# cgbur/llama2.zig

Measured on AMD Instinct MI355X. Metric: tokens/s (argmax, -t 0), higher is better.
Workload: dtype f32; 1 GPU; llama2-7b shape, fp32 llama2.c-v0 checkpoint (dim 4096, hidden 11008, L 32, H 32, kv 32, V 32000, S 2048), greedy from BOS, seeded synthetic weights; parallelism=1 GPU

## Files before the change

llama2.zig_amd/csrc/forward.cpp:

```cpp
#include <algorithm>
#include <cmath>
#include <cstdlib>
#include <cstring>
#include <mutex>

#include "batch_host.h"
#include "l2z_state.h"

namespace l2z {

struct Prof {
    std::vector<hipEvent_t> ev;
    std::vector<int> kind;
};

#define L2Z_LAUNCH(kind_id, expr)                                                         \
    do {                                                                                  \
        hipEvent_t _a = nullptr, _b = nullptr;                                            \
        if (prof) {                                                                       \
            L2Z_HIP(hipEventCreate(&_a));                                                 \
            L2Z_HIP(hipEventCreate(&_b));                                                 \
            L2Z_HIP(hipEventRecord(_a, st));                                              \
        }                                                                                 \
        L2Z_HIP(expr);                                                                    \
        if (prof) {                                                                       \
            L2Z_HIP(hipEventRecord(_b, st));                                              \
            prof->ev.push_back(_a);                                                       \
            prof->ev.push_back(_b);                                                       \
            prof->kind.push_back(kind_id);                                                \
        }                                                                                 \
    } while (0)

int check_pair(const l2z_config *config, const l2z_runstate *s, const l2z_weights *w, bool paged_ok)
{
    L2Z_CHECK(config && s && w, L2Z_ERR_INVALID, "null config / runstate / weights");
    L2Z_CHECK(paged_ok || s->pool == nullptr, L2Z_ERR_INVALID,
              "a paged runstate (l2z_runstate_init_paged) is taken by the wide family only: l2z_prefill_batch, "
              "l2z_transformer_wide, l2z_wide_run, l2z_verify_wide");
    L2Z_CHECK(memcmp(config, &s->cfg, sizeof *config) == 0 &&
                  memcmp(config, &w->cfg, sizeof *config) == 0,
              L2Z_ERR_INVALID, "config does not match the one RunState / Weights were built with");
    L2Z_CHECK(s->device == w->device && s->sh.rank == w->sh.rank && s->sh.world == w->sh.world,
              L2Z_ERR_INVALID, "RunState and Weights live on different devices / shards");
    L2Z_CHECK(s->sh.scheme_b == w->sh.scheme_b, L2Z_ERR_INVALID,
              "RunState and Weights were built under different sharding schemes (L2Z_SCHEME_B changed in between)");
    return L2Z_OK;
}

int enqueue_forward(l2z_runstate *s, const l2z_weights *w, StepKind step, Prof *prof,
                    int only_stage, int variant, int only_kind)
{
    const bool with_step = step != STEP_NONE;
    const bool split = variant == ATTN_SPLIT || variant == ATTN_SPLIT_S;
    const l2z_config &c = s->cfg;
    const Shard &sh = s->sh;
    hipStream_t st = s->stream;
    const l2z_comm *lc = s->comm;
    const size_t dim = c.dim, hid = c.hidden_dim;
    const int mb = s->max_blocks;
    int stage = 0;
    auto want = [&]() { return only_stage < 0 || only_stage == stage; };
    auto kind = [&](int k) { return only_kind < 0 || only_kind == k; };
    const bool p2p = s->d_push != nullptr && only_stage < 0 && sh.world > 1;
    const bool consume = p2p && s->ll_consume;
    const bool can_push = p2p && consume;
    const bool sb = sh.scheme_b;
    const bool xchg = step == STEP_GREEDY && p2p && s->xchg_steps;
    const int n_g = s->n_gathers;
    int gi = 0;
    bool pushed = false;
    const int *ctl = lc ? lc->d_ctl : nullptr;
    auto gather = [&](float *buf, size_t count_per_rank) -> int {
        stage++;
        gi++;
        if (only_stage >= 0 || only_kind >= 0) return L2Z_OK;
        const bool was_pushed = pushed;
        pushed = false;
        if (consume) {
            L2Z_CHECK(was_pushed, L2Z_ERR_STATE, "consumer-side gather %d: the producer did not push", gi);
            if (gi < n_g) return L2Z_OK;
        }
        hipEvent_t ea = nullptr, eb = nullptr;
        const bool timed = prof != nullptr && s->comm != nullptr && s->comm->world > 1;
        if (timed) {
            L2Z_HIP(hipEventCreate(&ea));
            L2Z_HIP(hipEventCreate(&eb));
            L2Z_HIP(hipEventRecord(ea, st));
        }
        L2Z_TRY(comm_allgather_inplace(s->comm, buf, count_per_rank, gi, n_g, was_pushed, st));
        if (timed) {
            L2Z_HIP(hipEventRecord(eb, st));
            prof->ev.push_back(ea);
            prof->ev.push_back(eb);
            prof->kind.push_back(KIND_GATHER);
        }
        return L2Z_OK;
    };
    auto reduce = [&]() -> int {
        stage++;
        gi++;
        if (only_stage >= 0 || only_kind >= 0) return L2Z_OK;
        const bool was_pushed = pushed;
        pushed = false;
        hipEvent_t ea = nullptr, eb = nullptr;
        if (prof != nullptr) {
            L2Z_HIP(hipEventCreate(&ea));
            L2Z_HIP(hipEventCreate(&eb));
            L2Z_HIP(hipEventRecord(ea, st));
        }
        L2Z_TRY(comm_allreduce(s->comm, s->part, s->x, dim, gi, was_pushed, st));
        if (prof != nullptr) {
            L2Z_HIP(hipEventRecord(eb, st));
            prof->ev.push_back(ea);
            prof->ev.push_back(eb);
            prof->kind.push_back(KIND_GATHER);
        }
        return L2Z_OK;
    };
    auto x_in = [&](MatvecArgs &a, const float *plain, int g, size_t count_per_rank) {
        a.x = plain;
        if (consume && g >= 1) a.xin = comm_ll_in(s->comm, g, count_per_rank);
    };
    auto push_to = [&](MatvecArgs &a, int which) {
        if (!can_push) return;
        a.push = s->d_push + which;
        a.push_ctl = ctl;
        a.push_gi = comm_gi(lc, gi + 1);
    };
    auto col_shard = [&](MatvecArgs &a, const float *wcols, const float *x_loc, int n_pad, int *epi) {
        a.w0 = wcols;
        a.x = x_loc;
        a.n = n_pad;
        a.rows0 = c.dim;
        a.out0 = s->part;
        a.resid = sh.rank == 0 ? s->x : nullptr;
        *epi = sh.rank == 0 ? EPI_RESID : EPI_STORE;
        push_to(a, 1);
    };
    const bool pk = s->packed_w && w->pk_blob != nullptr && !sb && sh.world == 1 && !consume;
    for (int l = 0; l < c.n_layers; l++) {
        float *kc = s->key_cache + (size_t)l * c.seq_len * sh.kvd_loc;
        float *vc = s->value_cache + (size_t)l * c.seq_len * sh.kvd_loc;
        const size_t kvh_stride = (size_t)c.seq_len * sh.hs;
        const bool fused = s->fused_qkv_attn && !split && only_stage < 0;
        if (fused && kind(KIND_QKV)) {
            FusedQkvAttnArgs a = {};
            a.wq = w->wq + (size_t)l * dim * dim;
            a.wk = w->wk + (size_t)l * dim * dim;
            a.wv = w->wv + (size_t)l * dim * dim;
            a.rms_w = w->rms_att + (size_t)l * dim; a.x = s->x; a.q_out = s->q;
            a.kcache = kc; a.vcache = vc; a.xb = s->xb; a.pos_ptr = s->d_pos; a.rope = s->rope;
            a.n = c.dim; a.head_size = sh.hs; a.seq_len = c.seq_len; a.kv_dim = sh.kvd_loc;
            a.kv_row = sh.hs; a.kv_head = kvh_stride;
            L2Z_LAUNCH(KIND_QKV, launch_fused_qkv_attn(a, c.n_heads, st));
        }
        if (!fused && want() && kind(KIND_QKV)) {
            MatvecArgs a = {};
            a.w0 = w->wq + (size_t)l * sh.dim_loc * dim;
            a.w1 = w->wk + (size_t)l * sh.kvd_loc * dim;
            a.w2 = w->wv + (size_t)l * sh.kvd_loc * dim;
            a.out0 = s->q; a.out1 = kc; a.out2 = vc;
            a.rows0 = sh.dim_loc; a.rows1 = sh.kvd_loc; a.rows2 = sh.kvd_loc;
            a.pos_stride1 = sh.hs; a.pos_stride2 = sh.hs; a.kv_head_stride = kvh_stride;
            a.n = c.dim; a.rms_w = w->rms_att + (size_t)l * dim;
            x_in(a, s->x, gi, sh.dim_loc);
            a.pos_ptr = s->d_pos; a.rope = s->rope; a.head_size = sh.hs; a.rope_segs = 2;
            L2Z_LAUNCH(KIND_QKV, launch_matvec(a, PRO_RMS, EPI_ROPE, mb, g_cus, st));
        }
        if (!fused && want() && kind(KIND_ATTN)) {
            AttnArgs a = {};
            a.q = s->q; a.kcache = kc; a.vcache = vc; a.xb = s->xb + sh.dim0;
            a.pos_ptr = s->d_pos; a.head_size = sh.hs; a.kv_row = sh.hs; a.kv_head = kvh_stride;
            a.kv_mul = c.n_heads / c.n_kv_heads; a.seq_len = c.seq_len;
            a.tl_seq = s->tl_attn_seq++;
            if (!sb && can_push && attention_push_supported(a)) {
                a.push = s->d_push + 0;
                a.push_ctl = ctl;
                a.push_gi = comm_gi(lc, gi + 1);
                pushed = true;
            }
            if (split && s->attn_nch > 1 && attention_split_supported(a))
                L2Z_LAUNCH(KIND_ATTN, launch_attention_split(a, sh.heads_loc, s->attn_nch,
                                                             s->d_attn_part, s->d_attn_cnt, st, variant == ATTN_SPLIT_S));
            else
                L2Z_LAUNCH(KIND_ATTN, launch_attention(a, sh.heads_loc, st, variant == ATTN_SHORT ? 1 : 0));
        }
        if (!sb) L2Z_TRY(gather(s->xb, sh.dim_loc));
        if (want() && kind(KIND_WO)) {
            MatvecArgs a = {};
            int epi = EPI_RESID;
            if (sb) {
                col_shard(a, w->wo + (size_t)l * dim * sh.dimc_pad, s->xb + sh.dim0, sh.dimc_pad, &epi);
            } else {
                a.w0 = w->wo + (size_t)l * sh.dim_loc * dim;
                a.out0 = s->x + sh.dim0; a.resid = s->x + sh.dim0;
                a.rows0 = sh.dim_loc; a.n = c.dim;
                x_in(a, s->xb, gi, sh.dim_loc);
                push_to(a, 1);
            }
            L2Z_LAUNCH(KIND_WO, launch_matvec(a, PRO_NONE, epi, mb, g_cus, st, nullptr, &pushed));
        }
        if (sb) L2Z_TRY(reduce());
        else L2Z_TRY(gather(s->x, sh.dim_loc));
        if (want() && kind(KIND_FFN13)) {
            MatvecArgs a = {};
            a.w0 = w->w1 + (size_t)l * sh.hid_loc * 2 * dim;
            a.w1 = w->w3 + (size_t)l * sh.hid_loc * 2 * dim;
            a.out0 = sb ? s->hb : s->hb + sh.hid0;
            a.rows0 = sh.hid_loc; a.rows1 = sh.hid_loc; a.n = c.dim;
            a.rms_w = w->rms_ffn + (size_t)l * dim;
            x_in(a, s->x, gi, sh.dim_loc);
            if (!sb) push_to(a, 2);
            if (pk && w->pk[l].p != nullptr) { a.pk = w->pk[l].p; a.pk_e = w->pk[l].e; }
            L2Z_LAUNCH(KIND_FFN13, launch_matvec(a, PRO_RMS, EPI_SWIGLU, mb, g_cus, st, nullptr, &pushed));
        }
        if (!sb) L2Z_TRY(gather(s->hb, sh.hid_loc));
        if (want() && kind(KIND_FFN2)) {
            MatvecArgs a = {};
            int epi = EPI_RESID;
            if (sb) {
                col_shard(a, w->w2 + (size_t)l * dim * sh.hidc_pad, s->hb, sh.hidc_pad, &epi);
            } else {
                a.w0 = w->w2 + (size_t)l * sh.dim_loc * hid;
                a.out0 = s->x + sh.dim0; a.resid = s->x + sh.dim0;
                a.rows0 = sh.dim_loc; a.n = c.hidden_dim;
                x_in(a, s->hb, gi, sh.hid_loc);
                push_to(a, 1);
            }
            L2Z_LAUNCH(KIND_FFN2, launch_matvec(a, PRO_NONE, epi, mb, g_cus, st, nullptr, &pushed));
        }
        if (sb) L2Z_TRY(reduce());
        else L2Z_TRY(gather(s->x, sh.dim_loc));
    }
    if (want() && kind(KIND_CLS)) {
        MatvecArgs a = {};
        a.w0 = w->wcls; a.out0 = s->logits + sh.v0;
        a.rows0 = sh.v_loc; a.n = c.dim; a.rms_w = w->rms_final;
        x_in(a, s->x, gi, sh.dim_loc);
        a.part_val = s->d_part_val; a.part_idx = s->d_part_idx; a.row_offset = sh.v0;
        const bool fuse = (sh.world == 1 || xchg || (only_kind >= 0 && with_step && s->comm && !s->comm->nccl && !s->comm->p2p)) &&
                          matvec_vector_width(c.dim);
        int grid = 0;
        if (!xchg) push_to(a, 3);
        L2Z_LAUNCH(KIND_CLS, launch_matvec(a, PRO_RMS, fuse ? EPI_ARGMAX : EPI_STORE, mb, g_cus, st,
                                           &grid, &pushed));
        s->n_part = fuse ? grid : 0;
        if (only_stage < 0 && only_kind < 0) (with_step ? s->n_part_step : s->n_part_fwd) = s->n_part;
    }
    if (xchg) {
        stage++;
        gi++;
        pushed = false;
        if (only_kind < 0) s->logits_partial = true;
    } else {
        L2Z_TRY(gather(s->logits, sh.v_loc));
    }
    if (step == STEP_GREEDY && want() && kind(KIND_ARGMAX)) {
        ArgmaxArgs a = {};
        a.logits = s->logits; a.vocab = c.vocab_size; a.token_ptr = s->d_token;
        if (s->n_part > 0) { a.part_val = s->d_part_val; a.part_idx = s->d_part_idx; a.n_part = s->n_part; }
        a.pos_ptr = s->d_pos; a.prompt = s->d_prompt; a.n_prompt_ptr = s->d_n_prompt;
        a.out_tokens = s->d_out_tokens; a.argmax_out = s->d_argmax; a.tok_emb = w->tok_emb;
        a.x = s->x; a.dim = c.dim; a.advance = 1;
        if (xchg && only_kind < 0) {
            a.xchg = s->d_push + 3;
            a.xchg_gi = comm_gi(lc, n_g);
            a.epoch_ctl = lc->d_ctl;
            a.epoch_add = lc->solo ? 0 : n_g;
        }
        L2Z_LAUNCH(KIND_ARGMAX, launch_argmax(a, st));
    }
    if (step == STEP_SAMPLE && want() && kind(KIND_ARGMAX)) {
        L2Z_CHECK(sh.world == 1 && s->d_smp_ctl != nullptr && s->d_smp_scratch != nullptr, L2Z_ERR_STATE,
                  "sampled step on a runstate l2z_sample_run has not prepared");
        SampleStepArgs a = {};
        a.logits = s->logits; a.vocab = c.vocab_size; a.seq_len = c.seq_len;
        a.params = (const SampleStepParams *)s->d_smp_ctl; a.coins = s->d_smp_ctl + 2; a.scratch = s->d_smp_scratch;
        a.token_ptr = s->d_token; a.pos_ptr = s->d_pos; a.prompt = s->d_prompt; a.n_prompt_ptr = s->d_n_prompt;
        a.out_tokens = s->d_out_tokens; a.tok_emb = w->tok_emb; a.x = s->x; a.dim = c.dim;
        L2Z_LAUNCH(KIND_ARGMAX, launch_sample_step(a, st));
    }
    return L2Z_OK;
}

int attn_variant(const l2z_runstate *s, int pos)
{
    if (s->attn_nch > 1 && pos >= s->attn_split_pos) return pos < s->attn_split_wide_pos ? ATTN_SPLIT_S : ATTN_SPLIT;
    return pos < s->attn_short_pos ? ATTN_SHORT : ATTN_HEAD;
}

int build_graph(l2z_runstate *s, const l2z_weights *w, StepKind step, int variant,
                hipGraphExec_t *out)
{
    hipGraph_t graph = nullptr;
    L2Z_HIP(hipStreamBeginCapture(s->stream, hipStreamCaptureModeThreadLocal));
    int rc = enqueue_forward(s, w, step, nullptr, -1, variant);
    hipError_t e = hipStreamEndCapture(s->stream, &graph);
    if (rc != L2Z_OK) {
        if (graph) (void)hipGraphDestroy(graph);
        return rc;
    }
    L2Z_HIP(e);
    e = hipGraphInstantiate(out, graph, nullptr, nullptr, 0);
    (void)hipGraphDestroy(graph);
    L2Z_HIP(e);
    return L2Z_OK;
}

void drop_graphs(l2z_runstate *s)
{
    for (int v = 0; v < ATTN_VARIANTS; v++) {
        if (s->g_forward[v]) { (void)hipGraphExecDestroy(s->g_forward[v]); s->g_forward[v] = nullptr; }
        if (s->g_step[v]) { (void)hipGraphExecDestroy(s->g_step[v]); s->g_step[v] = nullptr; }
        if (s->g_sample[v]) { (void)hipGraphExecDestroy(s->g_sample[v]); s->g_sample[v] = nullptr; }
    }
    s->graph_w_uid = 0;
}

hipGraphExec_t *graph_slot(l2z_runstate *s, StepKind step, int variant)
{
    return step == STEP_SAMPLE ? &s->g_sample[variant] : step == STEP_GREEDY ? &s->g_step[variant] : &s->g_forward[variant];
}

int ensure_graph(l2z_runstate *s, const l2z_weights *w, int variant, StepKind step)
{
    if (!s->use_graphs) return L2Z_OK;
    int rc = L2Z_OK;
    if (s->graph_w_uid != w->uid) {
        drop_graphs(s);
        s->graph_w_uid = w->uid;
        const int edges[] = {0, s->attn_short_pos, s->attn_split_pos, s->attn_split_wide_pos, s->cfg.seq_len};
        bool reach[ATTN_VARIANTS] = {};
        for (int e : edges)
            for (int p = e - 1; p <= e; p++)
                if (p >= 0 && p < s->cfg.seq_len) reach[attn_variant(s, p)] = true;
        for (int v = 0; v < ATTN_VARIANTS && rc == L2Z_OK; v++) {
            if (!reach[v]) continue;
            rc = build_graph(s, w, STEP_NONE, v, &s->g_forward[v]);
            if (rc == L2Z_OK) rc = build_graph(s, w, STEP_GREEDY, v, &s->g_step[v]);
        }
    }
    hipGraphExec_t *slot = graph_slot(s, step, variant);
    if (rc == L2Z_OK && *slot) return L2Z_OK;
    if (rc != L2Z_OK || build_graph(s, w, step, variant, slot) != L2Z_OK) {
        fprintf(stderr, "llama2_hip: hipGraph capture failed (%s); launching eagerly\n", l2z_last_error());
        drop_graphs(s);
        s->use_graphs = false;
        (void)hipGetLastError();
    }
    return L2Z_OK;
}

int run_forward(l2z_runstate *s, const l2z_weights *w, StepKind step, int pos)
{
    const bool with_step = step != STEP_NONE;
    const int variant = attn_variant(s, pos);
    L2Z_CHECK(s->sh.world == 1 || (s->comm && (s->comm->nccl || s->comm->p2p)), L2Z_ERR_STATE,
              "sharded runstate without a transport: connect the group (RCCL id or "
              "l2z_comm_p2p_export/_connect), or drive emulated ranks with l2z_emu_transformer");
    L2Z_TRY(comm_check(s->comm));
    L2Z_TRY(ensure_graph(s, w, variant, step));
    s->logits_partial = step == STEP_GREEDY && s->xchg_steps && s->d_push != nullptr && s->sh.world > 1;
    if (s->use_graphs) {
        s->n_part = with_step ? s->n_part_step : s->n_part_fwd;
        L2Z_HIP(hipGraphLaunch(*graph_slot(s, step, variant), s->stream));
        return L2Z_OK;
    }
    return enqueue_forward(s, w, step, nullptr, -1, variant);
}

int ensure_logits(l2z_runstate *s)
{
    if (!s->logits_partial) return L2Z_OK;
    L2Z_TRY(comm_allgather_inplace(s->comm, s->logits, (size_t)s->sh.v_loc, 1, 1, false, s->stream));
    s->logits_partial = false;
    s->n_part = 0;
    return L2Z_OK;
}


}

using namespace l2z;

extern "C" int l2z_transformer(int token, int pos, const l2z_config *config, l2z_runstate *s,
                               const l2z_weights *w)
{
    L2Z_TRY(check_pair(config, s, w));
    L2Z_CHECK(token >= 0 && token < config->vocab_size, L2Z_ERR_STATE, "token %d out of range", token);
    L2Z_CHECK(pos >= 0 && pos < config->seq_len, L2Z_ERR_STATE, "pos %d out of range [0,%d)", pos,
              config->seq_len);
    L2Z_HIP(hipSetDevice(s->device));
    L2Z_HIP(launch_set_state(token, pos, s->d_token, s->d_pos, w->tok_emb, s->x, config->dim,
                             s->stream));
    L2Z_TRY(run_forward(s, w, STEP_NONE, pos));
    s->host_pos = pos + 1;
    return L2Z_OK;
}

extern "C" int l2z_argmax(l2z_runstate *s, int *out_token)
{
    L2Z_CHECK(s && out_token, L2Z_ERR_INVALID, "l2z_argmax: null argument");
    L2Z_HIP(hipSetDevice(s->device));
    L2Z_TRY(ensure_logits(s));
    ArgmaxArgs a = {};
    a.logits = s->logits; a.vocab = s->cfg.vocab_size; a.argmax_out = s->d_argmax; a.advance = 0;
    if (s->n_part > 0) { a.part_val = s->d_part_val; a.part_idx = s->d_part_idx; a.n_part = s->n_part; }
    L2Z_HIP(launch_argmax(a, s->stream));
    L2Z_HIP(hipMemcpyAsync(out_token, s->d_argmax, sizeof(int), hipMemcpyDeviceToHost, s->stream));
    L2Z_HIP(hipStreamSynchronize(s->stream));
    return L2Z_OK;
}

extern "C" int l2z_logits_read(l2z_runstate *s, float *out_logits)
{
    L2Z_CHECK(s && out_logits, L2Z_ERR_INVALID, "l2z_logits_read: null argument");
    L2Z_HIP(hipSetDevice(s->device));
    L2Z_TRY(ensure_logits(s));
    L2Z_HIP(hipMemcpyAsync(out_logits, s->logits, (size_t)s->cfg.vocab_size * sizeof(float),
                           hipMemcpyDeviceToHost, s->stream));
    L2Z_HIP(hipStreamSynchronize(s->stream));
    L2Z_TRY(comm_check(s->comm));
    return L2Z_OK;
}

extern "C" int l2z_probs_read(l2z_runstate *s, float temperature, float *out_probs)
{
    L2Z_CHECK(s && out_probs, L2Z_ERR_INVALID, "l2z_probs_read: null argument");
    L2Z_CHECK(temperature > 0.0f, L2Z_ERR_INVALID, "l2z_probs_read: temperature %g (0 is the argmax path)", (double)temperature);
    L2Z_HIP(hipSetDevice(s->device));
    L2Z_TRY(ensure_logits(s));
    if (s->d_probs == nullptr) L2Z_HIP(hipMalloc(&s->d_probs, (size_t)s->cfg.vocab_size * sizeof(float)));
    L2Z_HIP(launch_probs(s->d_probs, s->logits, s->cfg.vocab_size, temperature, s->stream));
    const size_t bytes = (size_t)s->cfg.vocab_size * sizeof(float);
    if (s->h_stage == nullptr) L2Z_HIP(hipHostMalloc((void **)&s->h_stage, bytes, hipHostMallocDefault));
    L2Z_HIP(hipMemcpyAsync(s->h_stage, s->d_probs, bytes, hipMemcpyDeviceToHost, s->stream));
    L2Z_HIP(hipStreamSynchronize(s->stream));
    L2Z_TRY(comm_check(s->comm));
    memcpy(out_probs, s->h_stage, bytes);
    return L2Z_OK;
}

extern "C" int l2z_greedy_begin(l2z_runstate *s, const int32_t *prompt, int n_prompt)
{
    L2Z_CHECK(s != nullptr && n_prompt >= 0 && (n_prompt == 0 || prompt != nullptr),
              L2Z_ERR_INVALID, "l2z_greedy_begin: bad arguments");
    L2Z_CHECK(n_prompt <= s->cfg.seq_len, L2Z_ERR_INVALID, "prompt longer than seq_len");
    L2Z_CHECK(s->pool == nullptr, L2Z_ERR_INVALID, "l2z_greedy_begin: a paged runstate is taken by the wide family only");
    for (int i = 0; i < n_prompt; i++)
        L2Z_CHECK(prompt[i] >= 0 && prompt[i] < s->cfg.vocab_size, L2Z_ERR_INVALID,
                  "prompt[%d] = %d out of vocabulary", i, prompt[i]);
    L2Z_HIP(hipSetDevice(s->device));
    L2Z_HIP(hipStreamSynchronize(s->stream));
    if (n_prompt)
        L2Z_HIP(hipMemcpy(s->d_prompt, prompt, (size_t)n_prompt * sizeof(int), hipMemcpyHostToDevice));
    L2Z_HIP(hipMemcpy(s->d_n_prompt, &n_prompt, sizeof(int), hipMemcpyHostToDevice));
    s->h_prompt.assign(prompt, prompt + n_prompt);
    s->host_pos = 0;
    s->done = false;
    return L2Z_OK;
}

namespace l2z {
namespace {

int step_loop(const l2z_config *config, l2z_runstate *s, const l2z_weights *w, int n_steps, StepKind step,
              int32_t *out_tokens, int *out_n)
{
    *out_n = 0;
    L2Z_HIP(hipSetDevice(s->device));
    if (s->done) return L2Z_OK;
    int remaining = n_steps;
    if (remaining > config->seq_len - s->host_pos) remaining = config->seq_len - s->host_pos;
    if (remaining <= 0) return L2Z_OK;
    if (s->host_pos == 0) {
        L2Z_HIP(launch_set_state(1, 0, s->d_token, s->d_pos, w->tok_emb, s->x, config->dim,
                                 s->stream));
    }
    const int kChunk = 64;
    int produced = 0;
    const int np = (int)s->h_prompt.size();
    if (s->host_pos == 0 && np >= kPrefillMinPrompt && remaining >= np && prefill_enabled() &&
        prefill_usable(s) &&
        std::find(s->h_prompt.begin(), s->h_prompt.end(), 1) == s->h_prompt.end()) {
        std::vector<int32_t> in((size_t)np);
        in[0] = 1;
        for (int i = 1; i < np; i++) in[(size_t)i] = s->h_prompt[(size_t)i - 1];
        L2Z_TRY(prefill_tokens(s, w, in.data(), np, 0));
        L2Z_HIP(hipMemcpyAsync(s->d_out_tokens, s->d_prompt, (size_t)np * sizeof(int),
                               hipMemcpyDeviceToDevice, s->stream));
        L2Z_HIP(launch_set_state(s->h_prompt[(size_t)np - 1], np, s->d_token, s->d_pos, w->tok_emb,
                                 s->x, config->dim, s->stream));
        for (int i = 0; i < np; i++) out_tokens[i] = s->h_prompt[(size_t)i];
        produced = np;
        s->host_pos = np;
        remaining -= np;
    }
    while (remaining > 0 && !s->done) {
        const int n = remaining < kChunk ? remaining : kChunk;
        for (int i = 0; i < n; i++) L2Z_TRY(run_forward(s, w, step, s->host_pos + i));
        L2Z_HIP(hipMemcpyAsync(out_tokens + produced, s->d_out_tokens + s->host_pos,
                               (size_t)n * sizeof(int), hipMemcpyDeviceToHost, s->stream));
        L2Z_HIP(hipStreamSynchronize(s->stream));
        L2Z_TRY(comm_check(s->comm));
        int got = n;
        for (int i = 0; i < n; i++) {
            if (out_tokens[produced + i] == 1) {
                got = i + 1;
                s->done = true;
                break;
            }
        }
        produced += got;
        s->host_pos += got;
        remaining -= n;
    }
    *out_n = produced;
    return L2Z_OK;
}

}
}

extern "C" int l2z_greedy_run(const l2z_config *config, l2z_runstate *s, const l2z_weights *w,
                              int n_steps, int32_t *out_tokens, int *out_n)
{
    L2Z_TRY(check_pair(config, s, w));
    L2Z_CHECK(out_tokens && out_n && n_steps >= 0, L2Z_ERR_INVALID, "l2z_greedy_run: bad arguments");
    return step_loop(config, s, w, n_steps, STEP_GREEDY, out_tokens, out_n);
}

extern "C" int l2z_sample_run(const l2z_config *config, l2z_runstate *s, const l2z_weights *w, int n_steps,
                              float temperature, float top_p, const float *coins, int32_t *out_tokens, int *out_n)
{
    L2Z_TRY(no_device_check());
    L2Z_CHECK(out_tokens && out_n && n_steps >= 0, L2Z_ERR_INVALID, "l2z_sample_run: bad arguments");
    L2Z_TRY(check_pair(config, s, w));
    L2Z_CHECK(s->comm == nullptr && s->sh.world == 1, L2Z_ERR_INVALID,
              "l2z_sample_run: the runstate is a shard (a shard holds its own rows of the logits only)");
    L2Z_TRY(check_draw("l2z_sample_run", -1, temperature, top_p, coins));
    if (temperature > 0.0f) L2Z_TRY(check_coins("l2z_sample_run", coins, 0, n_steps));
    *out_n = 0;
    const int left = config->seq_len - s->host_pos;
    const int n = n_steps < left ? n_steps : left;
    if (s->done || n <= 0) return L2Z_OK;
    L2Z_HIP(hipSetDevice(s->device));
    const size_t ctl_bytes = (2 + (size_t)config->seq_len) * sizeof(float);
    if (s->d_smp_ctl == nullptr) {
        L2Z_HIP(hipMalloc((void **)&s->d_smp_ctl, ctl_bytes));
        L2Z_HIP(hipMemset(s->d_smp_ctl, 0, ctl_bytes));
    }
    if (s->h_smp_ctl == nullptr) L2Z_HIP(hipHostMalloc((void **)&s->h_smp_ctl, ctl_bytes, hipHostMallocDefault));
    if (s->d_smp_scratch == nullptr)
        L2Z_HIP(hipMalloc((void **)&s->d_smp_scratch, sample_scratch_floats(config->vocab_size) * sizeof(float)));
    s->h_smp_ctl[0] = temperature;
    s->h_smp_ctl[1] = top_p;
    L2Z_HIP(hipMemcpyAsync(s->d_smp_ctl, s->h_smp_ctl, 2 * sizeof(float), hipMemcpyHostToDevice, s->stream));
    if (temperature > 0.0f) {
        float *h = s->h_smp_ctl + 2 + s->host_pos;
        memcpy(h, coins, (size_t)n * sizeof(float));
        L2Z_HIP(hipMemcpyAsync(s->d_smp_ctl + 2 + s->host_pos, h, (size_t)n * sizeof(float), hipMemcpyHostToDevice, s->stream));
    }
    return step_loop(config, s, w, n_steps, STEP_SAMPLE, out_tokens, out_n);
}

extern "C" int l2z_profile_forward(int token, int pos, const l2z_config *config, l2z_runstate *s,
                                   const l2z_weights *w, double *ms_by_kind, int *launches_by_kind,
                                   int n_kinds)
{
    L2Z_TRY(check_pair(config, s, w));
    L2Z_CHECK(ms_by_kind && launches_by_kind && n_kinds >= KIND_COUNT, L2Z_ERR_INVALID,
              "l2z_profile_forward: need %d kind slots", (int)KIND_COUNT);
    L2Z_CHECK(token >= 0 && token < config->vocab_size && pos >= 0 && pos < config->seq_len,
              L2Z_ERR_STATE, "token/pos out of range");
    L2Z_HIP(hipSetDevice(s->device));
    L2Z_HIP(launch_set_state(token, pos, s->d_token, s->d_pos, w->tok_emb, s->x, config->dim,
                             s->stream));
    Prof prof;
    int rc = enqueue_forward(s, w, STEP_GREEDY, &prof, -1, attn_variant(s, pos));
    hipError_t e = hipStreamSynchronize(s->stream);
    for (int k = 0; k < n_kinds; k++) { ms_by_kind[k] = 0.0; launches_by_kind[k] = 0; }
    if (rc == L2Z_OK && e == hipSuccess) {
        for (size_t i = 0; i < prof.kind.size(); i++) {
            float ms = 0.0f;
            if (hipEventElapsedTime(&ms, prof.ev[2 * i], prof.ev[2 * i + 1]) == hipSuccess) {
                ms_by_kind[prof.kind[i]] += ms;
                launches_by_kind[prof.kind[i]] += 1;
            }
        }
    }
    for (hipEvent_t ev : prof.ev) (void)hipEventDestroy(ev);
    s->host_pos = pos + 1;
    if (rc != L2Z_OK) return rc;
    L2Z_HIP(e);
    return L2Z_OK;
}

extern "C" int l2z_time_kind(int kind, int pos, const l2z_config *config, l2z_runstate *s,
                             const l2z_weights *w, int reps, double *avg_ms_per_launch, int *launches)
{
    L2Z_TRY(check_pair(config, s, w));
    L2Z_CHECK(kind >= 0 && kind < KIND_GATHER && avg_ms_per_launch && reps >= 1, L2Z_ERR_INVALID,
              "l2z_time_kind: bad arguments");
    L2Z_CHECK(s->sh.world == 1 || (s->comm && ((!s->comm->nccl && !s->comm->p2p) || s->comm->solo)), L2Z_ERR_INVALID,
              "l2z_time_kind: unsharded runstates, emulated or solo ranks only (a connected shard would wait for its peers)");
    L2Z_CHECK(pos >= 0 && pos < config->seq_len, L2Z_ERR_STATE, "pos out of range");
    L2Z_HIP(hipSetDevice(s->device));
    L2Z_HIP(launch_set_state(1, pos, s->d_token, s->d_pos, w->tok_emb, s->x, config->dim, s->stream));
    hipEvent_t e0, e1;
    L2Z_HIP(hipEventCreate(&e0));
    L2Z_HIP(hipEventCreate(&e1));
    const int per_pass = kind == KIND_CLS || kind == KIND_ARGMAX ? 1 : config->n_layers;
    int rc = enqueue_forward(s, w, STEP_GREEDY, nullptr, -1, attn_variant(s, pos), kind);
    hipError_t e = hipEventRecord(e0, s->stream);
    for (int r = 0; r < reps && rc == L2Z_OK; r++) rc = enqueue_forward(s, w, STEP_GREEDY, nullptr, -1, attn_variant(s, pos), kind);
    if (e == hipSuccess) e = hipEventRecord(e1, s->stream);
    if (e == hipSuccess) e = hipEventSynchronize(e1);
    float ms = 0.0f;
    if (e == hipSuccess) e = hipEventElapsedTime(&ms, e0, e1);
    (void)hipEventDestroy(e0);
    (void)hipEventDestroy(e1);
    hipError_t e2 = launch_set_state(1, pos, s->d_token, s->d_pos, w->tok_emb, s->x, config->dim, s->stream);
    if (e2 == hipSuccess) e2 = hipStreamSynchronize(s->stream);
    if (rc != L2Z_OK) return rc;
    L2Z_HIP(e);
    L2Z_HIP(e2);
    *avg_ms_per_launch = (double)ms / (double)(reps * per_pass);
    if (launches) *launches = reps * per_pass;
    return L2Z_OK;
}

extern "C" int l2z_emu_transformer(int n_ranks, l2z_runstate *const *ss,
                                   const l2z_weights *const *ws, int token, int pos)
{
    L2Z_CHECK(n_ranks >= 1 && ss && ws, L2Z_ERR_INVALID, "l2z_emu_transformer: bad arguments");
    const l2z_config &c = ss[0]->cfg;
    for (int r = 0; r < n_ranks; r++) {
        L2Z_TRY(check_pair(&c, ss[r], ws[r]));
        L2Z_CHECK(ss[r]->sh.world == n_ranks && ss[r]->sh.rank == r, L2Z_ERR_INVALID,
                  "l2z_emu_transformer: runstate %d is not rank %d of %d", r, r, n_ranks);
        L2Z_HIP(launch_set_state(token, pos, ss[r]->d_token, ss[r]->d_pos, ws[r]->tok_emb, ss[r]->x,
                                 c.dim, ss[r]->stream));
    }
    const bool sb = ss[0]->sh.scheme_b;
    const int n_stages = (sb ? 2 : 4) * c.n_layers + 1;
    for (int stage = 0; stage < n_stages; stage++) {
        for (int r = 0; r < n_ranks; r++)
            L2Z_TRY(enqueue_forward(ss[r], ws[r], STEP_NONE, nullptr, stage, attn_variant(ss[r], pos)));
        for (int r = 0; r < n_ranks; r++) L2Z_HIP(hipStreamSynchronize(ss[r]->stream));
        if (sb && stage < n_stages - 1) {
            const float *parts[kMaxWorld];
            L2Z_CHECK(n_ranks <= kMaxWorld, L2Z_ERR_INVALID, "l2z_emu_transformer: more than %d ranks", kMaxWorld);
            for (int r = 0; r < n_ranks; r++) parts[r] = ss[r]->part;
            for (int r = 0; r < n_ranks; r++) L2Z_HIP(launch_sum_parts(ss[r]->x, parts, n_ranks, c.dim, nullptr));
            L2Z_HIP(hipDeviceSynchronize());
            continue;
        }
        const Shard &sh0 = ss[0]->sh;
        size_t count;
        int which;
        if (stage == n_stages - 1) { which = 3; count = sh0.v_loc; }
        else if (stage % 4 == 0) { which = 0; count = sh0.dim_loc; }
        else if (stage % 4 == 2) { which = 2; count = sh0.hid_loc; }
        else { which = 1; count = sh0.dim_loc; }
        auto buf = [&](l2z_runstate *s) {
            return which == 0 ? s->xb : which == 1 ? s->x : which == 2 ? s->hb : s->logits;
        };
        for (int src = 0; src < n_ranks; src++)
            for (int dst = 0; dst < n_ranks; dst++)
                if (dst != src)
                    L2Z_HIP(hipMemcpy(buf(ss[dst]) + (size_t)src * count,
                                      buf(ss[src]) + (size_t)src * count, count * sizeof(float),
                                      hipMemcpyDeviceToDevice));
        L2Z_HIP(hipDeviceSynchronize());
    }
    for (int r = 0; r < n_ranks; r++) ss[r]->host_pos = pos + 1;
    return L2Z_OK;
}

extern "C" int l2z_kind_name(int kind, char *out, size_t cap)
{
    L2Z_CHECK(kind >= 0 && kind < KIND_COUNT && out && cap, L2Z_ERR_INVALID, "l2z_kind_name: bad kind");
    snprintf(out, cap, "%s", kKindNames[kind]);
    return L2Z_OK;
}
```

llama2.zig_amd/csrc/l2z_internal.h:

```cpp
#pragma once

#include <hip/hip_runtime.h>

#include <cstdarg>
#include <cstdint>
#include <cstdio>
#include <string>
#include <vector>

#include "../../include/llama2_hip.h"
#include "../../include/llama2_hip_test.h"

namespace l2z {

struct P2pArgs;

struct LLIn {
    const unsigned long long *slots;
    unsigned slot_floats;
    unsigned count;
    int gi;
    int *ctl;
    int *h_err;
    long long timeout_ticks;
};

void set_error(const char *fmt, ...);

#define L2Z_HIP(expr)                                                                    \
    do {                                                                                 \
        hipError_t _e = (expr);                                                          \
        if (_e != hipSuccess) {                                                          \
            ::l2z::set_error("%s failed: %s (%s:%d)", #expr, hipGetErrorString(_e),      \
                             __FILE__, __LINE__);                                        \
            return _e == hipErrorOutOfMemory ? L2Z_ERR_OOM                               \
                   : (_e == hipErrorNoDevice || _e == hipErrorInvalidDevice)             \
                       ? L2Z_ERR_NO_DEVICE                                               \
                       : L2Z_ERR_HIP;                                                    \
        }                                                                                \
    } while (0)

#define L2Z_CHECK(cond, code, ...)          \
    do {                                    \
        if (!(cond)) {                      \
            ::l2z::set_error(__VA_ARGS__);  \
            return (code);                  \
        }                                   \
    } while (0)

#define L2Z_TRY(expr)              \
    do {                           \
        int _s = (expr);           \
        if (_s != L2Z_OK) return _s; \
    } while (0)

template <class Sig> class FnRef;
template <class R, class... Args> class FnRef<R(Args...)> {
  public:
    template <class F>
    FnRef(const F &f) : f_(&f), call_([](const void *p, Args... args) -> R { return (*(const F *)p)(args...); }) {}
    R operator()(Args... args) const { return call_(f_, args...); }

  private:
    const void *f_;
    R (*call_)(const void *, Args...);
};


enum Prologue { PRO_NONE = 0, PRO_RMS = 1 };
enum Epilogue { EPI_STORE = 0, EPI_ROPE = 1, EPI_RESID = 2, EPI_SWIGLU = 3, EPI_ARGMAX = 4 };

constexpr int kMaxSeg = 3;

struct ArgmaxArgs {
    const float *logits;
    int vocab;
    const float *part_val;
    const int *part_idx;
    int n_part;
    int *token_ptr;
    int *pos_ptr;
    const int *prompt;
    const int *n_prompt_ptr;
    int *out_tokens;
    int *argmax_out;
    const float *tok_emb;
    float *x;
    int dim;
    int advance;
    int *epoch_ctl;
    int epoch_add;
    const P2pArgs *xchg;
    int xchg_gi;
};

struct MatvecArgs {
    const float *w0, *w1, *w2;
    float *out0, *out1, *out2;
    int rows0, rows1, rows2;
    int pos_stride1, pos_stride2;
    size_t kv_head_stride;
    int n;
    const float *x;
    const float *rms_w;
    const float *resid;
    const int *pos_ptr;
    const float2 *rope;
    int head_size;
    int rope_segs;
    float *part_val;
    int *part_idx;
    int row_offset;
    const P2pArgs *push;
    const int *push_ctl;
    int push_gi;
    LLIn xin;
    const uint32_t *pk;
    int pk_e;
};

struct AttnArgs {
    const float *q;
    const float *kcache;
    const float *vcache;
    float *xb;
    const int *pos_ptr;
    int head_size;
    int kv_row;
    size_t kv_head;
    int kv_mul;
    int seq_len;
    const P2pArgs *push;
    const int *push_ctl;
    int push_gi;
    int tl_seq;
};


struct FusedQkvAttnArgs {
    const float *wq, *wk, *wv;
    const float *rms_w, *x;
    float *q_out;
    float *kcache, *vcache;
    float *xb;
    const int *pos_ptr;
    const float2 *rope;
    int n;
    int head_size, seq_len, kv_dim;
    int kv_row;
    size_t kv_head;
};
bool fused_qkv_attn_supported(int dim, int n_heads, int n_kv_heads, int seq_len, int n_cus);
hipError_t launch_fused_qkv_attn(const FusedQkvAttnArgs &a, int n_heads, hipStream_t st);

hipError_t launch_pk_stats(const float *m, size_t count, uint32_t *stats, hipStream_t st);
hipError_t launch_pk_pack(const float *m, int rows, int n, int e_base, uint32_t *pk, hipStream_t st);
hipError_t launch_pk_unpack(const uint32_t *pk, int rows, int n, int e_base, float *out, hipStream_t st);
hipError_t launch_matvec(const MatvecArgs &a, int pro, int epi, int max_blocks_per_cu, int n_cus,
                         hipStream_t st, int *out_grid = nullptr, bool *pushed = nullptr);
bool attention_push_supported(const AttnArgs &a);
int matvec_max_grid(int n_cus);
bool matvec_vector_width(int n);
hipError_t launch_stream_read(const float *p, size_t n_floats, float *out, int n_cus, hipStream_t st);
hipError_t launch_attention(const AttnArgs &a, int n_heads_local, hipStream_t st, int form = 0);
int attention_short_pos(int head_size, int seq_len);
int attention_split_chunks(int n_heads_local, int n_cus);
size_t attention_split_part_floats(int n_heads_local, int head_size, int nch);
bool attention_split_supported(const AttnArgs &a);
hipError_t launch_attention_split(const AttnArgs &a, int n_heads_local, int nch, float *part,
                                  int *arrivals, hipStream_t st, bool small = false);
int attention_split_wide_pos(int seq_len);
hipError_t launch_argmax(const ArgmaxArgs &a, hipStream_t st);
hipError_t launch_set_state(int token, int pos, int *token_ptr, int *pos_ptr, const float *tok_emb,
                            float *x, int dim, hipStream_t st);
hipError_t launch_rmsnorm(float *o, const float *x, const float *w, int n, hipStream_t st);
hipError_t launch_softmax(float *x, int n, hipStream_t st);
hipError_t launch_probs(float *probs, const float *logits, int n, float temperature, hipStream_t st);
hipError_t launch_dot(float *out, const float *x, const float *y, int n, hipStream_t st);
hipError_t launch_weighted_sum_rows(float *xout, int xout_len, const float *rows, int row_stride,
                                    const float *weights, int n_weights, hipStream_t st);
hipError_t launch_synth_fill(float *dst, uint64_t base_idx, uint64_t count, uint64_t seed,
                             float scale, float bias, hipStream_t st, uint64_t row_len = 0, uint64_t row_pitch = 0,
                             uint64_t idx_pitch = 0);
hipError_t launch_sum_parts(float *out, const float *const *parts, int n_parts, int n, hipStream_t st);
hipError_t launch_copy_rows(float *dst, size_t dpitch, const float *src, size_t rows, size_t cols, hipStream_t st);
size_t attention_lds_bytes(int head_size, int seq_len, bool vec);

struct SplitKWs {
    float *part;
    int *cnt;
    size_t part_floats;
    int cnt_ints;
    void *x3;
    size_t x3_bytes;
    void *x3b;
    size_t x3b_bytes;
};
struct DeferredSum {
    const float *part;
    int sk, feat, tm;
    bool valid;
};
enum PlanesReady { PLANES_SPLIT = 0, PLANES_READY = 1, PLANES_READY_B = 2 };
constexpr int kSplitKMaxTokens = 256;
constexpr int kPanelWsRows = 6 * kSplitKMaxTokens;
int prefill_split_k(long long n_whole, int P, int K, bool pair);
enum PrefillGemmEpi { PG_STORE = 0, PG_RESID = 1, PG_ROPE = 2, PG_ROPE_CACHE = 3, PG_CACHE = 4,
                      PG_SWIGLU = 5 };
bool x3_applies(long long n_whole, int K);
bool x3_stream_shape(long long n_whole, int P, int K);
int x3_stream_sk(long long n_whole, int P, int K);
enum GemmKind { GEMM_SINGLE = 0,
                GEMM_QKV,
                GEMM_W13,
                GEMM_KV };
struct GemmShape {
    int kind, epi;
    int P, N, K, ldx;
    int n_scale;
    long long n_launch_whole;
    int sk;
    int nq, nkv;
    int w13_one_matrix;
    size_t part_floats;
    int cnt_ints;
};
enum GemmFamily { GF_INVALID = -1, GF_NOT_SUPPORTED = -2, GF_NO_WORKSPACE = -3,
                  GF_STREAM = 1,
                  GF_SHORT,
                  GF_SPLIT_K,
                  GF_TWO_BLOCK,
                  GF_TILE };
enum TileForm { TILE_128x64 = 0, TILE_64x64, TILE_32x64, TILE_32x32, TILE_128x128 };
struct GemmPlan {
    int family;
    int epi;
    int K;
    int x3;
    int sk;
    int tile;
    int feat, tm, nbuf, one_round;
    int tms, paired;
};
GemmPlan prefill_gemm_plan(const GemmShape &s);
hipError_t launch_prefill_rmsnorm(float *o, int ldo, const float *x, const float *w, int n, int P,
                                  hipStream_t st,
                                  void *x3 = nullptr, int kp = 0,
                                  const DeferredSum *pending = nullptr,
                                  const int *rows = nullptr);
hipError_t launch_prefill_embed(float *x, const float *tok_emb, const int *tokens, int dim, int P,
                                hipStream_t st);
hipError_t launch_prefill_attention(const float *q, int ldq, const float *kcache, const float *vcache,
                                    float *out, int ldo, int pos0, int P, int n_heads, int head_size,
                                    int kv_row, size_t kv_head, int kv_mul, int seq_len, hipStream_t st,
                                    int n_heads_model = 0,
                                    int form = 0,
                                    void *x3 = nullptr, int kp = 0,
                                    bool *planes_written = nullptr);
constexpr int kRaggedMaxSeq = 16;
struct RaggedSeq {
    float *kc, *vc;
    int row0, rows;
    int pos0;
    int pad;
    const int32_t *pages;
};
__device__ __forceinline__ int kv_page_id(const int32_t *pages, int i)
{
    return ((const __attribute__((address_space(4))) int32_t *)pages)[i];
}
struct RaggedLayer {
    const float *q;
    int ldq;
    float *out;
    int ldo;
    int P, n_heads, head_size, kv_mul, seq_len;
    size_t layer_off, kv_head_stride;
    hipStream_t st;
    void *x3;
    int kp;
};
using RaggedAttention = FnRef<hipError_t(const RaggedLayer &, bool *planes_written)>;
struct RaggedChunk {
    const RaggedSeq *seq;
    const int *row_seq;
    const int *row_pos;
    const int2 *tiles;
    int n_seq, n_tiles;
    int seq_max;
    float *k, *v;
    size_t page_floats;
    const RaggedAttention *attention;
    const int *att_rows;
    int n_att_rows;
};
hipError_t launch_ragged_rope_scatter(float *q, int ldq, const RaggedChunk &rg, int P, int dim, int kv_dim, int head_size,
                                      const float2 *rope, size_t layer_off, size_t kv_head_stride, hipStream_t st);
hipError_t launch_ragged_attention(const RaggedLayer &L, const RaggedChunk &rg, bool *planes_written = nullptr);
enum PanelEpi { PANEL_STORE = 0, PANEL_RESID = 1, PANEL_SWIGLU = 2, PANEL_QKV = 3 };
struct PanelProduct {
    const float *x;
    int ldx;
    const float *w0, *w1, *w2;
    int rows0, rows1, rows2;
    int P, K;
    int mode;
    float *out;
    int ldo;
    const float *res;
    int ldres;
    float *outk, *outv;
    int ldkv, head_size, pos0;
    size_t kv_head_stride;
    const float2 *rope;
};
bool prefill_panel_shape(long long n_whole, int P, int K, long long widest_whole);
int prefill_panel_max_tokens();
int prefill_next_chunk_of(const l2z_config &c, int remaining);
hipError_t launch_prefill_panel(const PanelProduct &p, int n_cus, const SplitKWs *ws, hipStream_t st);
int prefill_tile_form(int N, int P, int pair);
constexpr int kScoreSeg = 4096;
struct ScoreArgs {
    const float *slab;
    int ld, n, col0, P;
    const int *targets;
    float *part_m, *part_s;
    int *part_i;
    float *tgt;
    int seg0, nseg;
    float *out_logprob;
    int *out_top1;
};
hipError_t launch_score_reduce(const ScoreArgs &a, hipStream_t st);
hipError_t launch_score_finish(const ScoreArgs &a, hipStream_t st);
size_t matvec_lds_bytes(int n);

}
```

llama2.zig_amd/csrc/l2z_state.h:

```cpp
#pragma once
#include <cstdint>
#include <vector>

#include "kv_pages.h"
#include "l2z_comm.h"
#include "l2z_internal.h"
#include "tunables.h"

namespace l2z {

struct BatchScratch;
struct WideScratch;

struct Shard {
    int rank = 0, world = 1;
    int hs = 0;
    int dim0 = 0, dim_loc = 0;
    int kvd_loc = 0;
    int heads_loc = 0;
    int hid0 = 0, hid_loc = 0;
    int v0 = 0, v_loc = 0;
    bool scheme_b = false;
    int dimc_pad = 0, hidc_pad = 0;
};
int pad_cols(int n);
int make_shard(const l2z_config &c, const l2z_comm *comm, Shard *out);

enum ShardKind { REPL, BY_Q_HEADS, BY_KV_HEADS, BY_HIDDEN, BY_DIM_ROWS, BY_VOCAB, SKIP };

struct TensorDesc {
    const char *name;
    size_t offset;
    size_t layers, rows, cols;
    ShardKind kind;
    float scale, bias;
    size_t count() const { return layers * rows * cols; }
};
std::vector<TensorDesc> tensor_table(const l2z_config &c, bool shared);
void shard_rows(const TensorDesc &d, const Shard &s, size_t *r0, size_t *r1);

extern int g_cus;
int ensure_device(int device);
int current_device_for(const l2z_comm *comm);

}

struct l2z_weights {
    uint64_t uid = 0;
    l2z_config cfg;
    int shared;
    int device;
    l2z::Shard sh;
    float *blob = nullptr;
    size_t blob_floats = 0;
    bool file_layout = false;
    std::vector<size_t> dev_off;
    const float *tok_emb = nullptr, *rms_att = nullptr, *rms_ffn = nullptr, *rms_final = nullptr;
    const float *wq = nullptr, *wk = nullptr, *wv = nullptr, *wo = nullptr;
    const float *w1 = nullptr, *w2 = nullptr, *w3 = nullptr, *wcls = nullptr;
    struct PkMat {
        const uint32_t *p = nullptr;
        int e = 0;
    };
    uint32_t *pk_blob = nullptr;
    std::vector<PkMat> pk;
    int pk_packed = 0, pk_candidates = 0;
};

struct l2z_kvpool {
    l2z_config cfg;
    int device = 0;
    l2z::KvPages alloc;
    float *k = nullptr, *v = nullptr;
    size_t page_floats = 0;
    int live = 0;
};

enum { KIND_QKV = 0, KIND_ATTN, KIND_WO, KIND_FFN13, KIND_FFN2, KIND_CLS, KIND_ARGMAX, KIND_GATHER, KIND_COUNT };
static const char *const kKindNames[KIND_COUNT] = {"qkv", "attn", "wo", "ffn13", "ffn2", "cls", "argmax", "gather"};
static_assert(KIND_COUNT == L2Z_N_KINDS, "include/llama2_hip_test.h L2Z_N_KINDS");

struct l2z_runstate {
    l2z_config cfg;
    int device;
    l2z::Shard sh;
    const l2z_comm *comm = nullptr;
    hipStream_t stream = nullptr;
    float *x = nullptr, *xb = nullptr, *hb = nullptr, *q = nullptr, *logits = nullptr;
    float *part = nullptr;
    float *key_cache = nullptr, *value_cache = nullptr;
    l2z_kvpool *pool = nullptr;
    l2z::KvSeq pg;
    int32_t *d_pages = nullptr, *h_pages = nullptr;
    bool pages_dirty = false;
    float2 *rope = nullptr;
    int *d_token = nullptr, *d_pos = nullptr, *d_prompt = nullptr, *d_n_prompt = nullptr;
    int *d_out_tokens = nullptr, *d_argmax = nullptr;
    float *pf_x = nullptr, *pf_xn = nullptr, *pf_q = nullptr, *pf_att = nullptr;
    float *pf_h1 = nullptr;
    int pf_ld_xn = 0, pf_ld_att = 0, pf_ld_h1 = 0;
    float *pf_stage = nullptr;
    float *pf_part = nullptr;
    int *pf_tokens = nullptr;
    l2z::DeferredSum pf_pending = {nullptr, 1, 128, 1, false};
    l2z::PlanesReady pf_planes_att = l2z::PLANES_SPLIT, pf_planes_h1 = l2z::PLANES_SPLIT;
    l2z::SplitKWs pf_sk = {nullptr, nullptr, 0, 0, nullptr, 0, nullptr, 0};
    int pf_cap = 0;
    void *sc_ws = nullptr, *sc_seq = nullptr;
    size_t sc_ws_bytes = 0;
    int sc_cap = 0, sc_slab_n = 0;
    int sc_slab_force = 0;
    float *d_probs = nullptr;
    float *h_stage = nullptr;
    float *d_smp_ctl = nullptr, *h_smp_ctl = nullptr, *d_smp_scratch = nullptr;
    float *d_part_val = nullptr;
    int *d_part_idx = nullptr;
    int n_part = 0;
    int n_part_step = 0, n_part_fwd = 0;
    float *d_attn_part = nullptr;
    int *d_attn_cnt = nullptr;
    int attn_nch = 0;
    int attn_split_pos = 0;
    int attn_short_pos = 0;
    int attn_split_wide_pos = 0;
    uint64_t graph_w_uid = 0;
    hipGraphExec_t g_forward[4] = {nullptr, nullptr, nullptr, nullptr}, g_step[4] = {nullptr, nullptr, nullptr, nullptr};
    hipGraphExec_t g_sample[4] = {nullptr, nullptr, nullptr, nullptr};
    bool use_graphs = true;
    int host_pos = 0;
    bool done = false;
    std::vector<int32_t> h_prompt;
    l2z::P2pArgs *d_push = nullptr;
    int n_gathers = 0;
    bool ll_consume = false;
    bool xchg_steps = false;
    bool logits_partial = false;
    bool fused_qkv_attn = false;
    int max_blocks = 0;
    bool packed_w = true;
    int tl_attn_seq = 0;
    l2z::BatchScratch *bt = nullptr;
    float *rg_k = nullptr, *rg_v = nullptr;
    void *rg_tab = nullptr;
    int rg_cap = 0;
    l2z::WideScratch *wd = nullptr;
};

namespace l2z {

struct Prof;
int check_pair(const l2z_config *config, const l2z_runstate *s, const l2z_weights *w, bool paged_ok = false);
enum { ATTN_SHORT = 0, ATTN_HEAD = 1, ATTN_SPLIT_S = 2, ATTN_SPLIT = 3, ATTN_VARIANTS = 4 };
enum StepKind { STEP_NONE = 0, STEP_GREEDY = 1, STEP_SAMPLE = 2 };
int enqueue_forward(l2z_runstate *s, const l2z_weights *w, StepKind step, Prof *prof, int only_stage,
                    int variant, int only_kind = -1);
int attn_variant(const l2z_runstate *s, int pos);
int run_forward(l2z_runstate *s, const l2z_weights *w, StepKind step, int pos);
int ensure_logits(l2z_runstate *s);
void drop_graphs(l2z_runstate *s);

constexpr int kPrefillMinPrompt = L2Z_PREFILL_MIN_PROMPT;
bool prefill_enabled();
bool prefill_usable(const l2z_runstate *s);
bool prefill_shard_takes_the_unsharded_kernels(const l2z_config &c, const Shard &sh);
int prefill_check(const l2z_config *config, const l2z_runstate *s);
struct ScoreCall;
int prefill_tokens(l2z_runstate *s, const l2z_weights *w, const int32_t *tokens, int n_tokens, int pos0,
                   const ScoreCall *score = nullptr);

int prefill_scratch(l2z_runstate *s, int need);
int prefill_ragged_chunk(l2z_runstate *s, const l2z_weights *w, const int32_t *tokens, int P, const RaggedChunk &rg);
int prefill_last_logits(l2z_runstate *s, const l2z_weights *w);
int prefill_rows_logits(l2z_runstate *s, const l2z_weights *w, int P, float *out, int ldo, const int *rows = nullptr);
int ragged_alloc(l2z_runstate *s, int need);

int kv_check_kind(const char *fn, int n, l2z_runstate *const *states);
int kv_attach(const char *fn, int n, l2z_runstate *const *states, const int32_t *pos0, const int32_t *counts, int count);
int kv_upload(int n, l2z_runstate *const *states, hipStream_t st);
void kv_seq_base(const l2z_runstate *s, RaggedSeq *q);
inline size_t kv_page_floats(const l2z_runstate *s) { return s->pool != nullptr ? s->pool->page_floats : 0; }
int kv_release(l2z_runstate *s, int n_pos);
int kv_copy_rows(l2z_runstate *dst, const l2z_runstate *src, int r0, int n_pos);
void kv_runstate_free(l2z_runstate *s);

void batch_free(l2z_runstate *s);
void wide_free(l2z_runstate *s);
const float *wide_verify_row(const l2z_runstate *s, int row);
void wide_verify_forget(l2z_runstate *s);

}
```

llama2.zig_amd/csrc/matvec.hip:

```cpp
#include <type_traits>

#include "argmax_rule.h"
#include "matvec_device.h"
#include "packed_w.h"

namespace l2z {
namespace {

__device__ __forceinline__ void dot2_scalar(const float *__restrict__ pa,
                                            const float *__restrict__ pb, const float *xs, int n,
                                            float &ra, float &rb)
{
    const int lane = threadIdx.x & 63;
    float sa = 0.0f, sb = 0.0f;
    for (int j = lane; j < n; j += kWave) {
        const float xv = xs[j];
        sa = fmaf(pa[j], xv, sa);
        sb = fmaf(pb[j], xv, sb);
    }
    ra = wave_sum(sa);
    rb = wave_sum(sb);
}

template <int LPR>
struct MvGeom {
    static constexpr int RW = kWave / LPR;
    static constexpr int U = (LPR == 64) ? 4 : 6;
};

template <int LPR>
__device__ __forceinline__ void mv_load(const float *pa, const float *pb, int c0, int n4,
                                        v4f (&wa)[MvGeom<LPR>::U], v4f (&wb)[MvGeom<LPR>::U])
{
    constexpr int U = MvGeom<LPR>::U;
    const v4f *a4 = (const v4f *)pa, *b4 = (const v4f *)pb;
#pragma unroll
    for (int k = 0; k < U; k++) {
        int c = c0 + LPR * k;
        c = c < n4 ? c : n4 - 1;
        wa[k] = ldg_nt(a4 + c);
        wb[k] = ldg_nt(b4 + c);
    }
}

template <int LPR>
__device__ __forceinline__ void mv_consume(const v4f *xs4, int c0, const v4f (&wa)[MvGeom<LPR>::U],
                                           const v4f (&wb)[MvGeom<LPR>::U], v4f &acc_a, v4f &acc_b)
{
    constexpr int U = MvGeom<LPR>::U;
#pragma unroll
    for (int k = 0; k < U; k++) {
        const v4f xv = xs4[c0 + LPR * k];
        acc_a = fma4(wa[k], xv, acc_a);
        acc_b = fma4(wb[k], xv, acc_b);
    }
}

struct MvStep {
    bool unit_done, more;
    int u_next, b_next;
};

__device__ __forceinline__ MvStep mv_step(int u, int b, int n_batches, int ustride, int n_units)
{
    MvStep s;
    s.unit_done = (b + 1 == n_batches);
    s.u_next = s.unit_done ? u + ustride : u;
    s.b_next = s.unit_done ? 0 : b + 1;
    s.more = s.u_next < n_units;
    return s;
}

template <int PRO, int EPI, int LPR, int XC, bool LL>
__global__ __launch_bounds__(kBlock) void matvec_kernel(const MatvecArgs a)
{
    using G = MvGeom<LPR>;
    constexpr int U = G::U, RW = G::RW;
    extern __shared__ __attribute__((aligned(16))) float lds[];
    const MvLocals m = mv_locals<EPI>(a);
    const int n4 = m.n >> 2;
    const int n_batches = (n4 + LPR * U - 1) / (LPR * U);
    const int n4_pad = n_batches * (LPR * U);
    float *xs = lds;
    float *scratch = lds + 4 * n4_pad;
    const v4f *xs4 = (const v4f *)xs;

    const int lane = threadIdx.x & 63, wave = threadIdx.x >> 6;
    const int grp = lane / LPR, cl = lane % LPR;
    const int n_units = (m.n_pairs + RW - 1) / RW;
    const int ustride = gridDim.x * kWaves;

    XStage<PRO, XC, LL> xst;
    xst.issue(a.x, a.xin, a.rms_w, n4);
    int u = blockIdx.x * kWaves + wave;
    const bool has_unit = u < n_units;
    const float *pa, *pb;
    pair_rows<EPI>(m, (has_unit ? u : 0) * RW + grp, pa, pb);
    v4f wa[U], wb[U];
    EpiIn ein = epi_prefetch<EPI>(m, (has_unit ? u : 0) * RW + grp, cl == 0 && has_unit);
    EpiIn ein_next = ein;
    mv_load<LPR>(pa, pb, cl, n4, wa, wb);
    xst.finish(a.x, a.rms_w, m.n, n4_pad, xs, scratch);
    if (EPI != EPI_ARGMAX && !has_unit) return;

    v4f acc_a = {0.f, 0.f, 0.f, 0.f}, acc_b = {0.f, 0.f, 0.f, 0.f};
    ArgmaxCand best;
    int b = 0;
    while (has_unit) {
        mv_consume<LPR>(xs4, cl + b * (LPR * U), wa, wb, acc_a, acc_b);
        const MvStep s = mv_step(u, b, n_batches, ustride, n_units);
        if (s.more) {
            if (s.unit_done) {
                pair_rows<EPI>(m, s.u_next * RW + grp, pa, pb);
                ein_next = epi_prefetch<EPI>(m, s.u_next * RW + grp, cl == 0);
            }
            mv_load<LPR>(pa, pb, cl + s.b_next * (LPR * U), n4, wa, wb);
        }
        if (s.unit_done) {
            const float sa = lanes_sum(hsum4(acc_a), LPR);
            const float sb = lanes_sum(hsum4(acc_b), LPR);
            pair_epilogue<EPI>(m, u * RW + grp, sa, sb, cl == 0, ein);
            ein = ein_next;
            if (EPI == EPI_ARGMAX) {
                const int ra_ = 2 * (u * RW + grp), rb_ = ra_ + 1;
                if (ra_ < m.total_rows) argmax_take(best, sa, ra_ + a.row_offset);
                if (rb_ < m.total_rows) argmax_take(best, sb, rb_ + a.row_offset);
            }
            acc_a = v4f{0.f, 0.f, 0.f, 0.f};
            acc_b = v4f{0.f, 0.f, 0.f, 0.f};
        }
        if (!s.more) break;
        u = s.u_next;
        b = s.b_next;
    }
    if (EPI == EPI_ARGMAX) {
        argmax_wave_fold(best);
        __syncthreads();
        if (lane == 0) {
            scratch[wave] = best.v;
            scratch[kWaves + wave] = __int_as_float(best.i);
        }
        __syncthreads();
        if (threadIdx.x == 0) {
            ArgmaxCand c = {scratch[0], __float_as_int(scratch[kWaves])};
            for (int w = 1; w < kWaves; w++) argmax_merge(c, scratch[w], __float_as_int(scratch[kWaves + w]));
            a.part_val[blockIdx.x] = c.v;
            a.part_idx[blockIdx.x] = c.i;
        }
    }
}

struct PkRaw {
    v4u q4[7];
    uint32_t q1[3];
};

__device__ __forceinline__ void pk_load_raw(const uint32_t *src, int lane, int s, PkRaw &r)
{
    const int q = pk::lane_dw(s) / 4, rem = pk::lane_dw(s) % 4;
#pragma unroll
    for (int i = 0; i < 7; i++)
        if (i < q) r.q4[i] = __builtin_nontemporal_load((const v4u *)(src + i * 256 + lane * 4));
#pragma unroll
    for (int i = 0; i < 3; i++)
        if (i < rem) r.q1[i] = __builtin_nontemporal_load(src + q * 256 + i * 64 + lane);
}

template <int S>
__device__ __forceinline__ void pk_decode_lane(const PkRaw &r, int e31, v4f (&wa)[4], v4f (&wb)[4])
{
    constexpr int N = pk::lane_dw(S), Q = N / 4;
    uint32_t d[N > 0 ? N : 1], t[8 * S > 0 ? 8 * S : 1];
#pragma unroll
    for (int i = 0; i < N; i++) {
        if (i < 4 * Q) {
            const v4u v = r.q4[i / 4];
            d[i] = (i % 4 == 0) ? v.x : (i % 4 == 1) ? v.y : (i % 4 == 2) ? v.z : v.w;
        } else {
            d[i] = r.q1[i - 4 * Q];
        }
    }
    pk::decode_lane_t<S>(d, t);
#pragma unroll
    for (int k = 0; k < 4; k++) {
        if (k < S) {
            wa[k] = v4f{__builtin_amdgcn_ldexpf(__uint_as_float(t[8 * k]), e31), __builtin_amdgcn_ldexpf(__uint_as_float(t[8 * k + 1]), e31),
                        __builtin_amdgcn_ldexpf(__uint_as_float(t[8 * k + 2]), e31), __builtin_amdgcn_ldexpf(__uint_as_float(t[8 * k + 3]), e31)};
            wb[k] = v4f{__builtin_amdgcn_ldexpf(__uint_as_float(t[8 * k + 4]), e31), __builtin_amdgcn_ldexpf(__uint_as_float(t[8 * k + 5]), e31),
                        __builtin_amdgcn_ldexpf(__uint_as_float(t[8 * k + 6]), e31), __builtin_amdgcn_ldexpf(__uint_as_float(t[8 * k + 7]), e31)};
        } else {
            wa[k] = v4f{0.f, 0.f, 0.f, 0.f};
            wb[k] = v4f{0.f, 0.f, 0.f, 0.f};
        }
    }
}

constexpr int kRowU = 4;

template <int EPI, int XC>
struct RowF32 {
    static constexpr bool kAhead = false;
    v4f wa[kRowU], wb[kRowU];
    const float *pa, *pb;
    int n4;

    __device__ __forceinline__ void init(const MvLocals &, int n4_, int) { n4 = n4_; }
    __device__ __forceinline__ void point(const MvLocals &m, int u) { pair_rows<EPI>(m, u, pa, pb); }
    __device__ __forceinline__ void issue(int b)
    {
        const int tid = threadIdx.x, cb = b * (kBlock * kRowU);
        const v4f *a4 = (const v4f *)pa + cb + tid, *b4 = (const v4f *)pb + cb + tid;
        const int wbase = cb + (tid & ~63);
#pragma unroll
        for (int k = 0; k < kRowU; k++) {
            const bool in_row = wbase + kBlock * k < n4;
            if (XC == 12 && !in_row) {
                wa[k] = v4f{0.f, 0.f, 0.f, 0.f};
                wb[k] = v4f{0.f, 0.f, 0.f, 0.f};
                continue;
            }
            const int off = in_row ? kBlock * k : -(cb + (tid & ~63));
            wa[k] = ldg_nt(a4 + off);
            wb[k] = ldg_nt(b4 + off);
        }
    }
    __device__ __forceinline__ void deliver() {}
};

template <int XC>
struct RowPacked {
    static constexpr bool kAhead = true;
    v4f wa[kRowU], wb[kRowU];
    PkRaw raw, nraw;
    int s_cur, s_nxt;
    const uint32_t *pp;
    size_t pdw, last_off;
    int e31, s_last, wave_u, n_batches;

    __device__ __forceinline__ void init(const MvLocals &m, int n4, int n_batches_)
    {
        n_batches = n_batches_;
        e31 = m.pk_e - 31;
        wave_u = __builtin_amdgcn_readfirstlane(threadIdx.x >> 6);
        pdw = pk::pair_dw(n4);
        last_off = pk::chunk_off(n4, n_batches - 1, wave_u);
        s_last = pk::steps(n4, n_batches - 1, wave_u);
    }
    __device__ __forceinline__ void point(const MvLocals &m, int u) { pp = pair_packed(m, u, pdw); }
    __device__ __forceinline__ void issue(int b)
    {
        const bool last = b + 1 == n_batches;
        const uint32_t *src = pp + (last ? last_off : (size_t)b * (4 * 64 * pk::kMaxLaneDw) + (size_t)wave_u * (64 * pk::kMaxLaneDw));
        s_nxt = (XC == 4 || !last) ? 4 : s_last;
        pk_load_raw(src, threadIdx.x & 63, XC == 4 ? 4 : s_nxt, nraw);
    }
    __device__ __forceinline__ void rotate()
    {
        raw = nraw;
        s_cur = s_nxt;
    }
    __device__ __forceinline__ void deliver()
    {
        if constexpr (XC == 4) {
            pk_decode_lane<4>(raw, e31, wa, wb);
        } else {
            switch (s_cur) {
                case 4: pk_decode_lane<4>(raw, e31, wa, wb); break;
                case 3: pk_decode_lane<3>(raw, e31, wa, wb); break;
                case 2: pk_decode_lane<2>(raw, e31, wa, wb); break;
                case 1: pk_decode_lane<1>(raw, e31, wa, wb); break;
                default: pk_decode_lane<0>(raw, e31, wa, wb); break;
            }
        }
    }
};

template <int PRO, int EPI, int XC, bool LL, bool PK = false>
__global__ __launch_bounds__(kBlock) void matvec_row_kernel(const MatvecArgs a)
{
    constexpr int U = kRowU;
    using Src = typename std::conditional<PK, RowPacked<XC>, RowF32<EPI, XC>>::type;
    extern __shared__ __attribute__((aligned(16))) float lds[];
    const MvLocals m = mv_locals<EPI>(a);
    const int n4 = m.n >> 2;
    const int n_batches = (n4 + kBlock * U - 1) / (kBlock * U);
    const int n4_pad = n_batches * (kBlock * U);
    float *xs = lds;
    float *scratch = lds + 4 * n4_pad;
    float *part = scratch + kScratch;
    const v4f *xs4 = (const v4f *)xs;
    const int tid = threadIdx.x, lane = tid & 63, wave = tid >> 6;
    const int n_units = m.n_pairs;
    const int ustride = gridDim.x;

    XStage<PRO, XC, LL> xst;
    xst.issue(a.x, a.xin, a.rms_w, n4);
    int u = blockIdx.x;
    Src src;
    src.init(m, n4, n_batches);
    src.point(m, u);
    EpiIn ein = epi_prefetch<EPI>(m, u, tid == 0);
    EpiIn ein_next = ein;
    src.issue(0);
    if constexpr (Src::kAhead) src.rotate();
    xst.finish(a.x, a.rms_w, m.n, n4_pad, xs, scratch);

    v4f acc_a = {0.f, 0.f, 0.f, 0.f}, acc_b = {0.f, 0.f, 0.f, 0.f};
    ArgmaxCand best;
    int b = 0, parity = 0;
    while (true) {
        const MvStep s = mv_step(u, b, n_batches, ustride, n_units);
        auto issue_next = [&]() __attribute__((always_inline)) {
            if (s.more) {
                if (s.unit_done) {
                    src.point(m, s.u_next);
                    ein_next = epi_prefetch<EPI>(m, s.u_next, tid == 0);
                }
                src.issue(s.b_next);
            }
        };
        if constexpr (Src::kAhead) issue_next();
        src.deliver();
#pragma unroll
        for (int k = 0; k < U; k++) {
            const v4f xv = xs4[b * (kBlock * U) + tid + kBlock * k];
            acc_a = fma4(src.wa[k], xv, acc_a);
            acc_b = fma4(src.wb[k], xv, acc_b);
        }
        if constexpr (!Src::kAhead) issue_next();
        if (s.unit_done) {
            const float sa = wave_sum(hsum4(acc_a));
            const float sb = wave_sum(hsum4(acc_b));
            float *pp_ = part + parity * (2 * kWaves);
            if (lane == 0) {
                pp_[wave] = sa;
                pp_[kWaves + wave] = sb;
            }
            __syncthreads();
            if (tid == 0) {
                const float ta = ((pp_[0] + pp_[1]) + pp_[2]) + pp_[3];
                const float tb = ((pp_[kWaves] + pp_[kWaves + 1]) + pp_[kWaves + 2]) + pp_[kWaves + 3];
                pair_epilogue<EPI>(m, u, ta, tb, true, ein);
                if (EPI == EPI_ARGMAX) {
                    const int ra_ = 2 * u, rb_ = ra_ + 1;
                    argmax_take(best, ta, ra_ + a.row_offset);
                    if (rb_ < m.total_rows) argmax_take(best, tb, rb_ + a.row_offset);
                }
            }
            ein = ein_next;
            parity ^= 1;
            acc_a = v4f{0.f, 0.f, 0.f, 0.f};
            acc_b = v4f{0.f, 0.f, 0.f, 0.f};
        }
        if (!s.more) break;
        if constexpr (Src::kAhead) src.rotate();
        u = s.u_next;
        b = s.b_next;
    }
    if (EPI == EPI_ARGMAX && tid == 0) {
        a.part_val[blockIdx.x] = best.v;
        a.part_idx[blockIdx.x] = best.i;
    }
}

template <int PRO, int EPI>
__global__ __launch_bounds__(kBlock) void matvec_scalar_kernel(const MatvecArgs a)
{
    extern __shared__ __attribute__((aligned(16))) float lds[];
    const MvLocals m = mv_locals<EPI>(a);
    float *xs = lds;
    float *scratch = lds + ((m.n + 3) & ~3);
    stage_x_scalar<PRO>(a.x, a.rms_w, m.n, xs, scratch);
    const int lane = threadIdx.x & 63, wave = threadIdx.x >> 6;
    for (int u = blockIdx.x * kWaves + wave; u < m.n_pairs; u += gridDim.x * kWaves) {
        const float *pa, *pb;
        pair_rows<EPI>(m, u, pa, pb);
        float sa, sb;
        dot2_scalar(pa, pb, xs, m.n, sa, sb);
        pair_epilogue<EPI>(m, u, sa, sb, lane == 0, epi_prefetch<EPI>(m, u, lane == 0));
    }
}

int lpr_for(int n4)
{
    int l = 8;
    while (l < 64 && l * 6 < n4) l <<= 1;
    return l;
}

struct MvLaunch {
    const void *fn;
    int lpr, u;
};

template <int PRO, int EPI, int LPR, int XC, bool LL>
MvLaunch mv_entry()
{
    return {reinterpret_cast<const void *>(&matvec_kernel<PRO, EPI, LPR, XC, LL>), LPR, MvGeom<LPR>::U};
}

template <int PRO, int EPI, bool LL>
MvLaunch mv_pick(int lpr, bool big_x)
{
    if (lpr == 8) return mv_entry<PRO, EPI, 8, 4, LL>();
    if (lpr == 16) return mv_entry<PRO, EPI, 16, 4, LL>();
    if (lpr == 32) return mv_entry<PRO, EPI, 32, 4, LL>();
    return big_x ? mv_entry<PRO, EPI, 64, 12, LL>() : mv_entry<PRO, EPI, 64, 4, LL>();
}

template <int PRO, int EPI, bool LL, bool PK = false>
const void *mv_row_fn(bool big_x)
{
    return big_x ? reinterpret_cast<const void *>(&matvec_row_kernel<PRO, EPI, 12, LL, PK>)
                 : reinterpret_cast<const void *>(&matvec_row_kernel<PRO, EPI, 4, LL, PK>);
}

#define L2Z_MV_COMBOS(X)                     \
    X(PRO_NONE, EPI_STORE,  0, 1, 0)         \
    X(PRO_NONE, EPI_RESID,  1, 1, 0)         \
    X(PRO_RMS,  EPI_STORE,  1, 1, 0)         \
    X(PRO_RMS,  EPI_ROPE,   1, 1, 0)         \
    X(PRO_RMS,  EPI_SWIGLU, 1, 1, 1)         \
    X(PRO_RMS,  EPI_ARGMAX, 1, 0, 0)
#define L2Z_IF_1(...) __VA_ARGS__
#define L2Z_IF_0(...)

const void *mv_row_pick_packed(int pro, int epi, bool big_x)
{
#define X(P, E, LL, SC, PK) L2Z_IF_##PK(if (pro == P && epi == E) return mv_row_fn<P, E, false, true>(big_x);)
    L2Z_MV_COMBOS(X)
#undef X
    return nullptr;
}

const void *mv_row_pick(int pro, int epi, bool big_x, bool ll)
{
#define X(P, E, LL, SC, PK)                                           \
    if (pro == P && epi == E && !ll) return mv_row_fn<P, E, false>(big_x); \
    L2Z_IF_##LL(if (pro == P && epi == E && ll) return mv_row_fn<P, E, true>(big_x);)
    L2Z_MV_COMBOS(X)
#undef X
    return nullptr;
}

MvLaunch mv_pick_pe(int pro, int epi, int lpr, bool big_x, bool vec, bool ll)
{
#define X(P, E, LL, SC, PK)                                                                \
    if (pro == P && epi == E && vec && !ll) return mv_pick<P, E, false>(lpr, big_x);       \
    L2Z_IF_##LL(if (pro == P && epi == E && vec && ll) return mv_pick<P, E, true>(lpr, big_x);) \
    L2Z_IF_##SC(if (pro == P && epi == E && !vec && !ll)                                   \
                    return MvLaunch{reinterpret_cast<const void *>(&matvec_scalar_kernel<P, E>), 0, 0};)
    L2Z_MV_COMBOS(X)
#undef X
    return {nullptr, 0, 0};
}
#undef L2Z_MV_COMBOS
#undef L2Z_IF_1
#undef L2Z_IF_0

__global__ __launch_bounds__(256) void stream_read_kernel(const v4f *__restrict__ p, size_t n4, float *out)
{
    constexpr int U = 8;
    size_t i = (size_t)blockIdx.x * 256 * U + threadIdx.x;
    const size_t stride = (size_t)gridDim.x * 256 * U;
    v4f acc = {0.f, 0.f, 0.f, 0.f};
    for (; i + 256 * (U - 1) < n4; i += stride) {
        v4f r[U];
#pragma unroll
        for (int k = 0; k < U; k++) r[k] = ldg_nt(p + i + 256 * k);
#pragma unroll
        for (int k = 0; k < U; k++) acc += r[k];
    }
    const float s = (acc.x + acc.y) + (acc.z + acc.w);
    if (s == 123.456f) out[blockIdx.x] = s;
}

}

size_t matvec_lds_bytes(int n) { return (size_t)(4 * ((n >> 2) + 1024) + kScratch + 4 * kWaves + 4) * sizeof(float); }

int matvec_max_grid(int n_cus) { return n_cus * 8; }

bool matvec_vector_width(int n) { return n > 0 && (n % 4) == 0; }

hipError_t launch_stream_read(const float *p, size_t n_floats, float *out, int n_cus, hipStream_t st)
{
    hipLaunchKernelGGL(stream_read_kernel, dim3(n_cus * 8), dim3(256), 0, st, (const v4f *)p, n_floats / 4, out);
    return hipGetLastError();
}

hipError_t launch_matvec(const MatvecArgs &a_in, int pro, int epi, int max_blocks_per_cu, int n_cus,
                         hipStream_t st, int *out_grid, bool *pushed)
{
    MatvecArgs a = a_in;
    if (max_blocks_per_cu > 8) max_blocks_per_cu = 8;
    bool vec = (a.n % 4) == 0 && aligned16(a.x) && aligned16(a.w0);
    if (a.rows1 > 0) vec = vec && aligned16(a.w1);
    if (a.rows2 > 0) vec = vec && aligned16(a.w2);
    if (pro == PRO_RMS) vec = vec && aligned16(a.rms_w);
    if (epi == EPI_SWIGLU && a.rows1 != a.rows0) return hipErrorInvalidValue;
    const int total_rows = a.rows0 + a.rows1 + a.rows2;
    const int n_pairs = (epi == EPI_SWIGLU) ? a.rows0 : (total_rows + 1) / 2;
    if (n_pairs <= 0 || a.n <= 0) return hipErrorInvalidValue;
    const int n4 = a.n >> 2;
    const int lpr = lpr_for(n4);
    if (epi == EPI_ARGMAX && (!vec || a.rows1 != 0 || a.rows2 != 0)) return hipErrorNotSupported;
    const Tunables &tn = tunables();
    const bool use_row = vec && n4 >= 1024 && (n4 % 64) == 0;
    const bool ll = a.xin.slots != nullptr;
    if (ll && !vec) return hipErrorNotSupported;
    if (a.pk != nullptr && (!use_row || ll || !pk::width_ok(a.n))) return hipErrorInvalidValue;
    MvLaunch k = {nullptr, 0, 0};
    size_t lds;
    int n_units;
    const auto padded = [n4](int batch) { return ((n4 + batch - 1) / batch) * batch; };
    if (use_row) {
        k.fn = a.pk != nullptr ? mv_row_pick_packed(pro, epi, a.n > 4096) : mv_row_pick(pro, epi, a.n > 4096, ll);
        lds = (size_t)(4 * padded(kBlock * kRowU) + kScratch + 4 * kWaves) * sizeof(float);
        n_units = n_pairs;
    } else if (vec) {
        k = mv_pick_pe(pro, epi, lpr, a.n > 4096, true, ll);
        if (k.fn == nullptr) return hipErrorInvalidValue;
        lds = (size_t)(4 * padded(k.lpr * k.u) + kScratch) * sizeof(float);
        const int rw = kWave / k.lpr;
        n_units = (n_pairs + rw - 1) / rw;
    } else {
        k = mv_pick_pe(pro, epi, lpr, a.n > 4096, false, ll);
        lds = (size_t)(((a.n + 3) & ~3) + kScratch) * sizeof(float);
        n_units = n_pairs;
    }
    if (k.fn == nullptr) return hipErrorInvalidValue;
    if (lds > 64 * 1024) {
        hipError_t e = hipFuncSetAttribute(k.fn, hipFuncAttributeMaxDynamicSharedMemorySize, (int)lds);
        if (e != hipSuccess) return e;
    }
    int occ = 0;
    if (hipOccupancyMaxActiveBlocksPerMultiprocessor(&occ, k.fn, kBlock, lds) != hipSuccess || occ < 1)
        occ = 1;
    if (occ > max_blocks_per_cu) occ = max_blocks_per_cu;
    if (use_row && occ > tn.row_blocks) occ = tn.row_blocks;
    int resident = occ * n_cus;
    if (tn.grid_cap > 0 && resident > tn.grid_cap) resident = tn.grid_cap;
    int grid;
    if (use_row) {
        grid = n_units;
        if (grid > resident) {
            const int per_block = (n_units + resident - 1) / resident;
            grid = (n_units + per_block - 1) / per_block;
        }
    } else {
        const int blocks_needed = (n_units + kWaves - 1) / kWaves;
        grid = blocks_needed;
        if (grid > resident) {
            const int per_wave = (n_units + resident * kWaves - 1) / (resident * kWaves);
            grid = (n_units + per_wave * kWaves - 1) / (per_wave * kWaves);
        }
    }
    if (out_grid) *out_grid = grid;
    if (!vec || epi == EPI_ROPE || a.rows2 != 0 || (epi != EPI_SWIGLU && a.rows1 != 0)) a.push = nullptr;
    if (pushed) *pushed = a.push != nullptr;
    void *args[] = {&a};
    return hipLaunchKernel(k.fn, dim3(grid), dim3(kBlock), args, lds, st);
}

}
```

llama2.zig_amd/csrc/matvec_device.h:

```cpp
#pragma once
#include "kernel_common.h"

namespace l2z {
namespace {

struct MvLocals {
    const float *w0, *w1, *w2;
    float *out0, *out1, *out2;
    const float *resid;
    const float2 *rope;
    int rows0, r01, total_rows, n_pairs, n, head_size, rope_segs, pos;
    size_t ps1, ps2;
    size_t kv_head_stride;
    const P2pArgs *push;
    int push_e;
    size_t push_base;
    const uint32_t *pk;
    int pk_e;
};

template <int EPI>
__device__ __forceinline__ MvLocals mv_locals(const MatvecArgs &a)
{
    MvLocals m;
    m.w0 = a.w0; m.w1 = a.w1; m.w2 = a.w2;
    m.out0 = a.out0; m.out1 = a.out1; m.out2 = a.out2;
    m.resid = a.resid; m.rope = a.rope;
    m.rows0 = a.rows0; m.r01 = a.rows0 + a.rows1; m.total_rows = a.rows0 + a.rows1 + a.rows2;
    m.n_pairs = (EPI == EPI_SWIGLU) ? a.rows0 : (m.total_rows + 1) >> 1;
    m.n = a.n; m.head_size = a.head_size; m.rope_segs = a.rope_segs;
    m.pos = (EPI == EPI_ROPE) ? *a.pos_ptr : 0;
    m.ps1 = (size_t)m.pos * (size_t)a.pos_stride1;
    m.ps2 = (size_t)m.pos * (size_t)a.pos_stride2;
    m.kv_head_stride = (EPI == EPI_ROPE) ? a.kv_head_stride : 0;
    m.push = a.push;
    m.push_e = m.push ? a.push_ctl[kCtlEpoch] + a.push_gi : 0;
    m.push_base = m.push ? (size_t)m.push->rank * m.push->count : 0;
    m.pk = a.pk; m.pk_e = a.pk_e;
    return m;
}

struct SegRow {
    bool past0, past1;
    int row;
    __device__ __forceinline__ int seg() const { return past1 ? 2 : (past0 ? 1 : 0); }
    template <typename T>
    __device__ __forceinline__ T pick(T v0, T v1, T v2) const
    {
        const T v = past0 ? v1 : v0;
        return past1 ? v2 : v;
    }
};

__device__ __forceinline__ SegRow seg_row(const MvLocals &m, int g)
{
    SegRow r;
    r.past0 = g >= m.rows0;
    r.past1 = g >= m.r01;
    r.row = g - (r.past1 ? m.r01 : (r.past0 ? m.rows0 : 0));
    return r;
}

template <int EPI>
__device__ __forceinline__ void pair_rows(const MvLocals &m, int p, const float *&pa, const float *&pb)
{
    if (p >= m.n_pairs) p = m.n_pairs - 1;
    if (EPI == EPI_SWIGLU) {
        pa = m.w0 + (size_t)(2 * p) * (size_t)m.n;
        pb = pa + m.n;
    } else {
        const int ga = 2 * p;
        const int gb = (ga + 1 < m.total_rows) ? ga + 1 : ga;
        const SegRow ra = seg_row(m, ga), rb = seg_row(m, gb);
        pa = ra.pick(m.w0, m.w1, m.w2) + (size_t)ra.row * (size_t)m.n;
        pb = rb.pick(m.w0, m.w1, m.w2) + (size_t)rb.row * (size_t)m.n;
    }
}

__device__ __forceinline__ const uint32_t *pair_packed(const MvLocals &m, int p, size_t pair_dw)
{
    if (p >= m.n_pairs) p = m.n_pairs - 1;
    return m.pk + (size_t)p * pair_dw;
}

struct EpiIn {
    float ra, rb;
    float2 cs;
};

template <int EPI>
__device__ __forceinline__ EpiIn epi_prefetch(const MvLocals &m, int p, bool writer)
{
    EpiIn e;
    e.ra = 0.0f; e.rb = 0.0f; e.cs = make_float2(1.0f, 0.0f);
    if (!writer || p >= m.n_pairs) return e;
    if (EPI == EPI_RESID) {
        const int ga = 2 * p, gb = ga + 1;
        e.ra = m.resid[ga];
        if (gb < m.total_rows) e.rb = m.resid[gb];
    } else if (EPI == EPI_ROPE) {
        const SegRow ra = seg_row(m, 2 * p);
        if (ra.seg() < m.rope_segs) {
            const int hs = m.head_size;
            e.cs = m.rope[(size_t)m.pos * (size_t)(hs >> 1) + (size_t)((ra.row % hs) >> 1)];
        }
    }
    return e;
}

template <int EPI>
__device__ __forceinline__ void pair_epilogue(const MvLocals &m, int p, float sa, float sb, bool writer, const EpiIn &in)
{
    const bool valid_a = p < m.n_pairs;
    if (EPI == EPI_SWIGLU) {
        float v = sa;
        v = v * (1.0f / (1.0f + expf(-v)));
        v = v * sb;
        if (writer && valid_a) {
            m.out0[p] = v;
            if (m.push) p2p_ll_push(m.push, m.push_e, m.push_base + (size_t)p, v);
        }
        return;
    }
    const int ga = 2 * p, gb = ga + 1;
    const bool valid_b = valid_a && gb < m.total_rows;
    const SegRow ra = seg_row(m, ga), rb = seg_row(m, gb);
    const int row_a = ra.row, row_b = rb.row;
    float *oa = ra.pick(m.out0, m.out1 + m.ps1, m.out2 + m.ps2);
    float *ob = rb.pick(m.out0, m.out1 + m.ps1, m.out2 + m.ps2);
    if (EPI == EPI_ROPE) {
        float o0 = sa, o1 = sb;
        if (ra.seg() < m.rope_segs) {
            const float2 cs = in.cs;
            o0 = sa * cs.x - sb * cs.y;
            o1 = sa * cs.y + sb * cs.x;
        }
        if (writer && valid_a) {
            size_t ia = (size_t)row_a, ib = (size_t)row_b;
            if (m.kv_head_stride) {
                const int hs = m.head_size;
                if (ra.past0) ia = (size_t)(row_a / hs) * m.kv_head_stride + (size_t)(row_a % hs);
                if (rb.past0) ib = (size_t)(row_b / hs) * m.kv_head_stride + (size_t)(row_b % hs);
            }
            oa[ia] = o0;
            if (valid_b) ob[ib] = o1;
        }
    } else if (EPI == EPI_RESID) {
        if (writer && valid_a) {
            const float va = in.ra + sa, vb = in.rb + sb;
            oa[row_a] = va;
            if (valid_b) ob[row_b] = vb;
            if (m.push) {
                p2p_ll_push(m.push, m.push_e, m.push_base + (size_t)row_a, va);
                if (valid_b) p2p_ll_push(m.push, m.push_e, m.push_base + (size_t)row_b, vb);
            }
        }
    } else {
        if (writer && valid_a) {
            oa[row_a] = sa;
            if (valid_b) ob[row_b] = sb;
            if (m.push) {
                p2p_ll_push(m.push, m.push_e, m.push_base + (size_t)row_a, sa);
                if (valid_b) p2p_ll_push(m.push, m.push_e, m.push_base + (size_t)row_b, sb);
            }
        }
    }
}

}
}
```

llama2.zig_amd/csrc/runstate.cpp:

```cpp
#include <algorithm>
#include <cmath>
#include <cstdlib>
#include <cstring>
#include <mutex>
#include <vector>

#include "l2z_state.h"

using namespace l2z;

static int runstate_make(const l2z_config *config, const l2z_comm *comm, l2z_kvpool *pool, l2z_runstate **out)
{
    L2Z_CHECK(config != nullptr && out != nullptr, L2Z_ERR_INVALID, "runstate_init: null argument");
    const int dev = current_device_for(comm);
    L2Z_TRY(ensure_device(dev));
    Shard sh;
    L2Z_TRY(make_shard(*config, comm, &sh));
    const l2z_config &c = *config;
    const size_t att_lds = attention_lds_bytes(sh.hs, c.seq_len, sh.hs % 4 == 0 && sh.kvd_loc % 4 == 0);
    L2Z_CHECK(att_lds <= 160 * 1024, L2Z_ERR_INVALID,
              "seq_len %d needs %zu bytes of LDS for attention scores (max 163840)", c.seq_len,
              att_lds);
    const int n_max = c.dim > c.hidden_dim ? c.dim : c.hidden_dim;
    L2Z_CHECK(matvec_lds_bytes(n_max) <= 160 * 1024, L2Z_ERR_INVALID,
              "dim/hidden_dim %d does not fit the 160 KiB LDS x-staging buffer", n_max);

    l2z_runstate *s = new l2z_runstate();
    s->cfg = c;
    s->device = dev;
    s->sh = sh;
    s->comm = comm;
    const Tunables &tn = tunables();
    s->max_blocks = tn.max_blocks_per_cu;
    s->use_graphs = tn.no_graph == 0;
    s->packed_w = tn.packed_w != 0;
    if (comm && comm->world > 1 && !comm->nccl && !comm->p2p) s->use_graphs = false;
    s->fused_qkv_attn = sh.world == 1 && tn.fuse_small != 0 &&
                        fused_qkv_attn_supported(c.dim, c.n_heads, c.n_kv_heads, c.seq_len, g_cus);
    s->n_gathers = (sh.scheme_b ? 2 : 4) * c.n_layers + 1;
    if (comm_uses_p2p(comm)) {
        const size_t longest = std::max((size_t)std::max(std::max(c.dim, c.hidden_dim), c.vocab_size),
                                        sh.scheme_b ? (size_t)sh.world * (size_t)c.dim : (size_t)0);
        if (comm->slot_floats < longest) {
            set_error("peer-write landing slots hold %zu floats, this config gathers up to %zu: pass "
                      "max(dim, hidden_dim, vocab_size%s) to l2z_comm_p2p_export", comm->slot_floats, longest,
                      sh.scheme_b ? ", world * dim" : "");
            delete s;
            return L2Z_ERR_COMM;
        }
    }

    const size_t kv = (size_t)c.n_layers * c.seq_len * sh.kvd_loc;
    hipError_t e = hipStreamCreateWithFlags(&s->stream, hipStreamNonBlocking);
    auto alloc = [&](void **p, size_t bytes) {
        if (e == hipSuccess) e = hipMalloc(p, bytes ? bytes : 4);
        if (e == hipSuccess) e = hipMemset(*p, 0, bytes ? bytes : 4);
    };
    alloc((void **)&s->x, (size_t)c.dim * 4);
    alloc((void **)&s->xb, ((size_t)c.dim + 256) * 4);
    alloc((void **)&s->hb, ((size_t)c.hidden_dim + 256) * 4);
    if (sh.scheme_b) alloc((void **)&s->part, (size_t)c.dim * 4);
    alloc((void **)&s->q, (size_t)c.dim * 4);
    alloc((void **)&s->logits, (size_t)c.vocab_size * 4);
    if (pool == nullptr) {
        alloc((void **)&s->key_cache, kv * 4);
        alloc((void **)&s->value_cache, kv * 4);
    } else {
        s->pg.init(c.seq_len);
        alloc((void **)&s->d_pages, s->pg.pages.size() * 4);
        if (e == hipSuccess) e = hipHostMalloc((void **)&s->h_pages, s->pg.pages.size() * 4, hipHostMallocDefault);
        s->pages_dirty = true;
    }
    alloc((void **)&s->rope, (size_t)c.seq_len * (sh.hs / 2) * sizeof(float2));
    alloc((void **)&s->d_token, 4);
    alloc((void **)&s->d_pos, 4);
    alloc((void **)&s->d_n_prompt, 4);
    alloc((void **)&s->d_argmax, 4);
    alloc((void **)&s->d_prompt, (size_t)c.seq_len * 4);
    alloc((void **)&s->d_out_tokens, (size_t)c.seq_len * 4);
    alloc((void **)&s->d_part_val, (size_t)matvec_max_grid(g_cus) * 4);
    alloc((void **)&s->d_part_idx, (size_t)matvec_max_grid(g_cus) * 4);
    {
        const int mode = tn.attn_split;
        int nch = mode > 0 ? mode : attention_split_chunks(c.n_heads, g_cus);
        if (nch > 16) nch = 16;
        s->attn_split_pos = mode > 0 ? 0 : 256;
        if (tn.attn_split_pos >= 0) s->attn_split_pos = tn.attn_split_pos;
        if (mode == 0 || c.seq_len <= s->attn_split_pos) nch = 0;
        s->attn_split_wide_pos = attention_split_wide_pos(c.seq_len);
        s->attn_short_pos = attention_short_pos(sh.hs, c.seq_len);
        if (nch > 1 && s->attn_short_pos > s->attn_split_pos) s->attn_short_pos = s->attn_split_pos;
        if (nch > 1) {
            s->attn_nch = nch;
            alloc((void **)&s->d_attn_part, attention_split_part_floats(sh.heads_loc, sh.hs, nch) * 4);
            alloc((void **)&s->d_attn_cnt, (size_t)sh.heads_loc * 4);
        }
    }
    if (comm_uses_p2p(comm) && e == hipSuccess) {
        AttnArgs aa = {};
        aa.q = s->q; aa.kcache = s->key_cache; aa.vcache = s->value_cache;
        aa.head_size = sh.hs; aa.kv_row = sh.hs; aa.kv_head = (size_t)c.seq_len * sh.hs;
        const bool want_consume = tn.p2p_consume >= 0 ? tn.p2p_consume != 0 : (sh.world <= 2 || c.dim < 4096);
        s->ll_consume = !sh.scheme_b && want_consume && matvec_vector_width(c.dim) &&
                        matvec_vector_width(c.hidden_dim) && attention_push_supported(aa);
        P2pArgs t[4];
        comm_p2p_args(comm, s->xb, (size_t)sh.dim_loc, s->ll_consume, &t[0]);
        comm_p2p_args(comm, sh.scheme_b ? s->part : s->x, sh.scheme_b ? (size_t)c.dim : (size_t)sh.dim_loc, s->ll_consume, &t[1]);
        comm_p2p_args(comm, s->hb, (size_t)sh.hid_loc, s->ll_consume, &t[2]);
        comm_p2p_args(comm, s->logits, (size_t)sh.v_loc, false, &t[3]);
        alloc((void **)&s->d_push, sizeof t);
        if (e == hipSuccess) e = hipMemcpy(s->d_push, t, sizeof t, hipMemcpyHostToDevice);
        s->xchg_steps = tn.argmax_xchg != 0 && matvec_vector_width(c.dim) && sh.v_loc >= 2 && comm->slot_floats >= 2 * (size_t)sh.world;
    }
    if (e != hipSuccess) {
        set_error("RunState allocation failed: %s", hipGetErrorString(e));
        l2z_runstate_free(s);
        return e == hipErrorOutOfMemory ? L2Z_ERR_OOM : L2Z_ERR_HIP;
    }
    {
        const int half = sh.hs / 2;
        std::vector<float2> tab((size_t)c.seq_len * half);
        for (int j = 0; j < half; j++) {
            const float head_dim = (float)(2 * j);
            const float freq = 1.0f / powf(10000.0f, head_dim / (float)sh.hs);
            for (int p = 0; p < c.seq_len; p++) {
                const float val = (float)p * freq;
                tab[(size_t)p * half + j] = make_float2(cosf(val), sinf(val));
            }
        }
        e = hipMemcpy(s->rope, tab.data(), tab.size() * sizeof(float2), hipMemcpyHostToDevice);
        if (e != hipSuccess) {
            set_error("RoPE table upload failed: %s", hipGetErrorString(e));
            l2z_runstate_free(s);
            return L2Z_ERR_HIP;
        }
    }
    if (pool != nullptr) {
        s->pool = pool;
        pool->live++;
    }
    *out = s;
    return L2Z_OK;
}

extern "C" int l2z_runstate_init(const l2z_config *config, const l2z_comm *comm, l2z_runstate **out)
{
    return runstate_make(config, comm, nullptr, out);
}

extern "C" int l2z_runstate_init_paged(const l2z_config *config, l2z_kvpool *pool, l2z_runstate **out)
{
    L2Z_CHECK(config != nullptr && pool != nullptr && out != nullptr, L2Z_ERR_INVALID, "l2z_runstate_init_paged: null argument");
    L2Z_CHECK(memcmp(config, &pool->cfg, sizeof *config) == 0, L2Z_ERR_INVALID,
              "l2z_runstate_init_paged: the pool was made with another config");
    L2Z_CHECK(current_device_for(nullptr) == pool->device, L2Z_ERR_INVALID,
              "l2z_runstate_init_paged: the pool lives on device %d, the current device is another", pool->device);
    return runstate_make(config, nullptr, pool, out);
}

extern "C" void l2z_runstate_free(l2z_runstate *s)
{
    if (!s) return;
    (void)hipSetDevice(s->device);
    if (s->stream) (void)hipStreamSynchronize(s->stream);
    for (int v = 0; v < l2z::ATTN_VARIANTS; v++) {
        if (s->g_forward[v]) (void)hipGraphExecDestroy(s->g_forward[v]);
        if (s->g_step[v]) (void)hipGraphExecDestroy(s->g_step[v]);
        if (s->g_sample[v]) (void)hipGraphExecDestroy(s->g_sample[v]);
    }
    void *ptrs[] = {s->x, s->xb, s->hb, s->q, s->logits, s->key_cache, s->value_cache, s->rope,
                    s->d_token, s->d_pos, s->d_prompt, s->d_n_prompt, s->d_out_tokens, s->d_argmax,
                    s->d_probs, s->d_part_val, s->d_part_idx, s->d_attn_part, s->d_attn_cnt, s->pf_x, s->pf_xn, s->pf_q,
                    s->pf_att, s->pf_h1, s->pf_stage, s->pf_part, s->pf_tokens, s->d_push, s->pf_sk.part, s->pf_sk.cnt, s->pf_sk.x3, s->pf_sk.x3b, s->part, s->sc_ws, s->sc_seq,
                    s->rg_k, s->rg_v, s->rg_tab, s->d_smp_ctl, s->d_smp_scratch};
    for (void *p : ptrs)
        if (p) (void)hipFree(p);
    if (s->h_stage) (void)hipHostFree(s->h_stage);
    if (s->h_smp_ctl) (void)hipHostFree(s->h_smp_ctl);
    if (s->pool == nullptr) {
        if (s->d_pages) (void)hipFree(s->d_pages);
        if (s->h_pages) (void)hipHostFree(s->h_pages);
    }
    l2z::kv_runstate_free(s);
    l2z::batch_free(s);
    l2z::wide_free(s);
    if (s->stream) (void)hipStreamDestroy(s->stream);
    delete s;
}

extern "C" int l2z_runstate_form(const l2z_runstate *s, int *form)
{
    L2Z_CHECK(s != nullptr && form != nullptr, L2Z_ERR_INVALID, "l2z_runstate_form: bad arguments");
    *form = s->sh.scheme_b ? 8 : 0;
    return L2Z_OK;
}

extern "C" int l2z_runstate_read(l2z_runstate *s, const char *name, size_t offset, size_t count,
                                 float *out)
{
    L2Z_CHECK(s && name && out, L2Z_ERR_INVALID, "l2z_runstate_read: null argument");
    const l2z_config &c = s->cfg;
    const size_t kv = (size_t)c.n_layers * c.seq_len * s->sh.kvd_loc;
    const float *p = nullptr;
    size_t n = 0;
    const std::string k = name;
    if (k == "x") { p = s->x; n = c.dim; }
    else if (k == "xb") { p = s->xb; n = c.dim; }
    else if (k == "hb") { p = s->hb; n = c.hidden_dim; }
    else if (k == "q") { p = s->q; n = c.dim; }
    else if (k == "logits") { p = s->logits; n = c.vocab_size; }
    else if (k == "key_cache") { p = s->key_cache; n = kv; }
    else if (k == "value_cache") { p = s->value_cache; n = kv; }
    const bool paged_kv = s->pool != nullptr && (k == "key_cache" || k == "value_cache");
    if (paged_kv) p = k == "key_cache" ? s->pool->k : s->pool->v;
    L2Z_CHECK(p != nullptr, L2Z_ERR_INVALID, "l2z_runstate_read: unknown buffer '%s'", name);
    L2Z_CHECK(offset + count <= n, L2Z_ERR_INVALID, "l2z_runstate_read: out of range");
    L2Z_HIP(hipSetDevice(s->device));
    if (k == "logits") L2Z_TRY(ensure_logits(s));
    L2Z_HIP(hipStreamSynchronize(s->stream));
    if (k == "key_cache" || k == "value_cache") {
        const size_t S = (size_t)c.seq_len, kvd = (size_t)s->sh.kvd_loc, hs = (size_t)s->sh.hs, layer = S * kvd;
        std::vector<float> host(layer);
        for (size_t l = offset / layer; l * layer < offset + count; l++) {
            if (paged_kv) {
                std::fill(host.begin(), host.end(), 0.0f);
                const size_t P = (size_t)l2z::kKvPage, run = P * hs;
                for (size_t pg = 0; pg < s->pg.pages.size(); pg++) {
                    if (s->pg.pages[pg] < 0) continue;
                    const size_t rows = std::min(P, S - pg * P);
                    L2Z_HIP(hipMemcpy2D(host.data() + pg * run, S * hs * 4,
                                        p + (size_t)s->pg.pages[pg] * s->pool->page_floats + l * (kvd / hs) * run, run * 4,
                                        rows * hs * 4, kvd / hs, hipMemcpyDeviceToHost));
                }
            } else
                L2Z_HIP(hipMemcpy(host.data(), p + l * layer, layer * sizeof(float), hipMemcpyDeviceToHost));
            const size_t lo = std::max(offset, l * layer), hi = std::min(offset + count, (l + 1) * layer);
            for (size_t i = lo; i < hi; i++) {
                const size_t r = i - l * layer, t = r / kvd, f = r % kvd;
                out[i - offset] = host[(f / hs) * S * hs + t * hs + f % hs];
            }
        }
        return L2Z_OK;
    }
    L2Z_HIP(hipMemcpy(out, p + offset, count * sizeof(float), hipMemcpyDeviceToHost));
    return L2Z_OK;
}

extern "C" int l2z_stream_read_probe(l2z_runstate *s, const l2z_weights *w, size_t slice_bytes, int reps,
                                     double *avg_gbps, double *best_gbps)
{
    L2Z_CHECK(s && w && avg_gbps && best_gbps && reps >= 1, L2Z_ERR_INVALID,
              "l2z_stream_read_probe: bad arguments");
    L2Z_HIP(hipSetDevice(s->device));
    const size_t blob_bytes = w->blob_floats * sizeof(float);
    if (slice_bytes == 0 || slice_bytes > blob_bytes) slice_bytes = blob_bytes;
    slice_bytes &= ~(size_t)4095;
    L2Z_CHECK(slice_bytes >= (1u << 20), L2Z_ERR_INVALID, "l2z_stream_read_probe: blob too small");
    const size_t n_slices = blob_bytes / slice_bytes;
    hipEvent_t e0, e1;
    L2Z_HIP(hipEventCreate(&e0));
    L2Z_HIP(hipEventCreate(&e1));
    double tot = 0.0, best = 1e30;
    int rc = L2Z_OK;
    for (int r = 0; r < reps + 2 && rc == L2Z_OK; r++) {
        const float *p = w->blob + (size_t)(r % n_slices) * (slice_bytes / sizeof(float));
        hipError_t e = hipEventRecord(e0, s->stream);
        if (e == hipSuccess) e = launch_stream_read(p, slice_bytes / sizeof(float), s->d_part_val, g_cus, s->stream);
        if (e == hipSuccess) e = hipEventRecord(e1, s->stream);
        if (e == hipSuccess) e = hipEventSynchronize(e1);
        float ms = 0.f;
        if (e == hipSuccess) e = hipEventElapsedTime(&ms, e0, e1);
        if (e != hipSuccess) {
            set_error("l2z_stream_read_probe: %s", hipGetErrorString(e));
            rc = L2Z_ERR_HIP;
            break;
        }
        if (r >= 2) {
            tot += ms;
            if (ms < best) best = ms;
        }
    }
    (void)hipEventDestroy(e0);
    (void)hipEventDestroy(e1);
    if (rc != L2Z_OK) return rc;
    *avg_gbps = (double)slice_bytes / (tot / reps * 1e-3) / 1e9;
    *best_gbps = (double)slice_bytes / (best * 1e-3) / 1e9;
    return L2Z_OK;
}

extern "C" int l2z_d2d_copy_probe(l2z_runstate *s, const l2z_weights *w, size_t slice_bytes, int reps,
                                  double *avg_gbps, double *best_gbps)
{
    L2Z_CHECK(s && w && avg_gbps && best_gbps && reps >= 1, L2Z_ERR_INVALID, "l2z_d2d_copy_probe: bad arguments");
    L2Z_HIP(hipSetDevice(s->device));
    const size_t blob_bytes = w->blob_floats * sizeof(float);
    if (slice_bytes == 0 || slice_bytes > blob_bytes) slice_bytes = blob_bytes;
    slice_bytes &= ~(size_t)4095;
    L2Z_CHECK(slice_bytes >= (1u << 20), L2Z_ERR_INVALID, "l2z_d2d_copy_probe: blob too small");
    const size_t n_slices = blob_bytes / slice_bytes;
    void *dst = nullptr;
    L2Z_HIP(hipMalloc(&dst, slice_bytes));
    hipEvent_t e0 = nullptr, e1 = nullptr;
    hipError_t e = hipEventCreate(&e0);
    if (e == hipSuccess) e = hipEventCreate(&e1);
    double tot = 0.0, best = 1e30;
    for (int r = 0; r < reps + 2 && e == hipSuccess; r++) {
        const float *p = w->blob + (size_t)(r % n_slices) * (slice_bytes / sizeof(float));
        e = hipEventRecord(e0, s->stream);
        if (e == hipSuccess) e = hipMemcpyAsync(dst, p, slice_bytes, hipMemcpyDeviceToDevice, s->stream);
        if (e == hipSuccess) e = hipEventRecord(e1, s->stream);
        if (e == hipSuccess) e = hipEventSynchronize(e1);
        float ms = 0.f;
        if (e == hipSuccess) e = hipEventElapsedTime(&ms, e0, e1);
        if (e == hipSuccess && r >= 2) {
            tot += ms;
            if (ms < best) best = ms;
        }
    }
    if (e0) (void)hipEventDestroy(e0);
    if (e1) (void)hipEventDestroy(e1);
    (void)hipFree(dst);
    if (e != hipSuccess) {
        set_error("l2z_d2d_copy_probe: %s", hipGetErrorString(e));
        return L2Z_ERR_HIP;
    }
    *avg_gbps = (double)slice_bytes / (tot / reps * 1e-3) / 1e9;
    *best_gbps = (double)slice_bytes / (best * 1e-3) / 1e9;
    return L2Z_OK;
}

extern "C" int l2z_synchronize(l2z_runstate *s)
{
    L2Z_CHECK(s != nullptr, L2Z_ERR_INVALID, "l2z_synchronize: null runstate");
    L2Z_HIP(hipSetDevice(s->device));
    L2Z_HIP(hipStreamSynchronize(s->stream));
    L2Z_TRY(comm_check(s->comm));
    return L2Z_OK;
}
```

llama2.zig_amd/csrc/tunables.cpp:

```cpp
#include "tunables.h"

#include <cstdlib>
#include <cstring>

namespace l2z {
namespace {

void env_int(const char *name, int *v)
{
    if (const char *e = getenv(name))
        if (*e) *v = atoi(e);
}

Tunables read_env()
{
    Tunables t;
    env_int("L2Z_GRID_CAP", &t.grid_cap);
    env_int("L2Z_ATTN_SPLIT", &t.attn_split);
    env_int("L2Z_ATTN_SPLIT_POS", &t.attn_split_pos);
    env_int("L2Z_FUSE_SMALL", &t.fuse_small);
    env_int("L2Z_SCHEME_B", &t.scheme_b);
    env_int("L2Z_NO_GRAPH", &t.no_graph);
    if (const char *e = getenv("L2Z_COMM")) t.prefer_rccl = strcmp(e, "rccl") == 0;
    env_int("L2Z_ARGMAX_XCHG", &t.argmax_xchg);
    env_int("L2Z_P2P_CONSUME", &t.p2p_consume);
    if (const char *e = getenv("L2Z_P2P_TIMEOUT_S"))
        if (*e) t.p2p_timeout_s = atoll(e);
    env_int("L2Z_P2P_BULK_MB", &t.p2p_bulk_mb);
    env_int("L2Z_PREFILL", &t.prefill);
    env_int("L2Z_PF_CHUNK", &t.pf_chunk);
    env_int("L2Z_PF_PANEL", &t.pf_panel);
    env_int("L2Z_PF_PANEL_MAX", &t.pf_panel_max);
    env_int("L2Z_PF_X3", &t.pf_x3);
    env_int("L2Z_PF_X3_STREAM_MIN", &t.pf_x3_stream_min);
    env_int("L2Z_PF_FUSE_PLANES", &t.pf_fuse_planes);
    env_int("L2Z_PACKED_W", &t.packed_w);
    return t;
}

}

namespace {
Tunables &mutable_tunables()
{
    static Tunables t = read_env();
    return t;
}
}

const Tunables &tunables() { return mutable_tunables(); }

int prefill_chunk_tokens()
{
    int n = tunables().pf_chunk > 0 ? tunables().pf_chunk : 1024;
    if (n < 16) n = 16;
    if (n > 2048) n = 2048;
    return n;
}

int prefill_next_chunk(int remaining)
{
    if (tunables().pf_chunk > 0) return remaining < prefill_chunk_tokens() ? remaining : prefill_chunk_tokens();
    return remaining >= 1024 ? 1024 : remaining < 512 ? remaining : 512;
}

bool tunables_set(const char *name, long long v)
{
    Tunables &t = mutable_tunables();
    struct { const char *n; int *p; } ints[] = {
        {"L2Z_GRID_CAP", &t.grid_cap}, {"L2Z_ATTN_SPLIT", &t.attn_split}, {"L2Z_ATTN_SPLIT_POS", &t.attn_split_pos},
        {"L2Z_FUSE_SMALL", &t.fuse_small}, {"L2Z_NO_GRAPH", &t.no_graph}, {"L2Z_SCHEME_B", &t.scheme_b},
        {"L2Z_COMM_RCCL", &t.prefer_rccl}, {"L2Z_ARGMAX_XCHG", &t.argmax_xchg}, {"L2Z_P2P_CONSUME", &t.p2p_consume},
        {"L2Z_P2P_BULK_MB", &t.p2p_bulk_mb}, {"L2Z_PREFILL", &t.prefill}, {"L2Z_PF_CHUNK", &t.pf_chunk},
        {"L2Z_PF_PANEL", &t.pf_panel}, {"L2Z_PF_PANEL_MAX", &t.pf_panel_max},
        {"L2Z_PF_X3", &t.pf_x3}, {"L2Z_PF_X3_STREAM_MIN", &t.pf_x3_stream_min},
        {"L2Z_PF_FUSE_PLANES", &t.pf_fuse_planes}, {"L2Z_PACKED_W", &t.packed_w}};
    for (auto &e : ints)
        if (strcmp(e.n, name) == 0) {
            *e.p = (int)v;
            return true;
        }
    if (strcmp(name, "L2Z_P2P_TIMEOUT_S") == 0) {
        t.p2p_timeout_s = v;
        return true;
    }
    return false;
}

}
```

llama2.zig_amd/csrc/tunables.h:

```cpp
#pragma once

namespace l2z {

struct Tunables {
    int grid_cap = 0;
    int attn_split = -1;
    int attn_split_pos = -1;
    int fuse_small = 1;
    int no_graph = 0;
    int prefer_rccl = 0;
    int p2p_consume = -1;
    int argmax_xchg = 1;
    long long p2p_timeout_s = 20;
    int scheme_b = 0;
    int p2p_bulk_mb = -1;
    int prefill = 1;
    int pf_chunk = 0;
    int pf_panel = 1;
    int pf_x3 = 1;
    int pf_x3_stream_min = 33;
    int pf_fuse_planes = 1;
    int packed_w = 1;
    int pf_panel_max = -1;

    static constexpr int row_blocks = 2;
    static constexpr int max_blocks_per_cu = 8;
    static constexpr int p2p_push = 1;
    static constexpr int reduce_block = 128;
    static constexpr int pf_skinny_max = 64;
};

const Tunables &tunables();
int prefill_chunk_tokens();
int prefill_next_chunk(int remaining);
bool tunables_set(const char *env_name, long long value);

}
```

llama2.zig_amd/csrc/weights.cpp:

```cpp
#include <algorithm>
#include <atomic>
#include <cmath>
#include <cstdlib>
#include <cstring>
#include <mutex>

#include "l2z_state.h"
#include "packed_w.h"
#include "tunables.h"

namespace l2z {

static thread_local char g_err[512] = "";

void set_error(const char *fmt, ...)
{
    va_list ap;
    va_start(ap, fmt);
    vsnprintf(g_err, sizeof g_err, fmt, ap);
    va_end(ap);
}

int make_shard(const l2z_config &c, const l2z_comm *comm, Shard *out)
{
    Shard s;
    s.rank = comm ? comm->rank : 0;
    s.world = comm ? comm->world : 1;
    L2Z_CHECK(c.dim > 0 && c.hidden_dim > 0 && c.n_layers > 0 && c.n_heads > 0 &&
                  c.n_kv_heads > 0 && c.vocab_size > 0 && c.seq_len > 0,
              L2Z_ERR_INVALID, "config: all seven fields must be positive");
    L2Z_CHECK(c.dim % c.n_heads == 0, L2Z_ERR_INVALID, "config: dim %% n_heads != 0");
    L2Z_CHECK(c.n_heads % c.n_kv_heads == 0, L2Z_ERR_INVALID, "config: n_heads %% n_kv_heads != 0");
    s.hs = c.dim / c.n_heads;
    L2Z_CHECK(s.hs % 2 == 0, L2Z_ERR_INVALID, "config: head_size must be even (RoPE pairs)");
    const int kv_dim = (int)(((int64_t)c.dim * c.n_kv_heads) / c.n_heads);
    int64_t a, b;
    L2Z_TRY(l2z_shard_range(c.dim, s.hs, s.rank, s.world, &a, &b));
    s.dim0 = (int)a;
    s.dim_loc = (int)(b - a);
    s.heads_loc = s.dim_loc / s.hs;
    L2Z_TRY(l2z_shard_range(kv_dim, s.hs, s.rank, s.world, &a, &b));
    s.kvd_loc = (int)(b - a);
    L2Z_TRY(l2z_shard_range(c.hidden_dim, 1, s.rank, s.world, &a, &b));
    s.hid0 = (int)a;
    s.hid_loc = (int)(b - a);
    L2Z_TRY(l2z_shard_range(c.vocab_size, 1, s.rank, s.world, &a, &b));
    s.v0 = (int)a;
    s.v_loc = (int)(b - a);
    s.scheme_b = tunables().scheme_b != 0 && comm != nullptr && (s.world > 1 || comm->nccl != nullptr);
    s.dimc_pad = pad_cols(s.dim_loc);
    s.hidc_pad = pad_cols(s.hid_loc);
    *out = s;
    return L2Z_OK;
}

int pad_cols(int n)
{
    const int n4 = (n + 3) / 4;
    return n > 768 ? ((n4 + 63) / 64) * 256 : n4 * 4;
}

std::vector<TensorDesc> tensor_table(const l2z_config &c, bool shared)
{
    const size_t V = c.vocab_size, dim = c.dim, hid = c.hidden_dim, L = c.n_layers;
    const size_t S = c.seq_len, hs = dim / c.n_heads, kvd = (dim * c.n_kv_heads) / c.n_heads;
    const float s_dim = sqrtf(3.0f / (float)dim), s_hid = sqrtf(3.0f / (float)hid);
    const float s_emb = 2.0f * s_dim;
    std::vector<TensorDesc> t = {
        {"token_embedding_table", 0, 1, V, dim, REPL, s_emb, 0.0f},
        {"rms_att_weight", 0, L, 1, dim, REPL, 0.1f, 1.0f},
        {"wq", 0, L, dim, dim, BY_Q_HEADS, s_dim, 0.0f},
        {"wk", 0, L, kvd, dim, BY_KV_HEADS, s_dim, 0.0f},
        {"wv", 0, L, kvd, dim, BY_KV_HEADS, s_dim, 0.0f},
        {"wo", 0, L, dim, dim, BY_DIM_ROWS, s_dim, 0.0f},
        {"rms_ffn_weight", 0, L, 1, dim, REPL, 0.1f, 1.0f},
        {"w1", 0, L, hid, dim, BY_HIDDEN, s_dim, 0.0f},
        {"w2", 0, L, dim, hid, BY_DIM_ROWS, s_hid, 0.0f},
        {"w3", 0, L, hid, dim, BY_HIDDEN, s_dim, 0.0f},
        {"rms_final_weight", 0, 1, 1, dim, REPL, 0.1f, 1.0f},
        {"freq_cis_real", 0, 1, 1, S * hs / 2, SKIP, 1.0f, 0.0f},
        {"freq_cis_imag", 0, 1, 1, S * hs / 2, SKIP, 1.0f, 0.0f},
    };
    if (!shared) t.push_back({"wcls", 0, 1, V, dim, BY_VOCAB, s_emb, 0.0f});
    size_t off = 0;
    for (auto &d : t) {
        d.offset = off;
        off += d.count();
    }
    return t;
}

void shard_rows(const TensorDesc &d, const Shard &s, size_t *r0, size_t *r1)
{
    switch (d.kind) {
        case BY_Q_HEADS:
        case BY_DIM_ROWS: *r0 = s.dim0; *r1 = (size_t)s.dim0 + s.dim_loc; break;
        case BY_KV_HEADS: *r0 = (size_t)s.rank * s.kvd_loc; *r1 = *r0 + s.kvd_loc; break;
        case BY_HIDDEN: *r0 = s.hid0; *r1 = (size_t)s.hid0 + s.hid_loc; break;
        case BY_VOCAB: *r0 = s.v0; *r1 = (size_t)s.v0 + s.v_loc; break;
        default: *r0 = 0; *r1 = d.rows; break;
    }
}

int g_cus = 0;

int ensure_device(int device)
{
    int n = 0;
    hipError_t e = hipGetDeviceCount(&n);
    if (e != hipSuccess || n <= 0) {
        set_error("no HIP device available (%s); this library has no CPU fallback",
                  e == hipSuccess ? "device count is 0" : hipGetErrorString(e));
        return L2Z_ERR_NO_DEVICE;
    }
    L2Z_CHECK(device >= 0 && device < n, L2Z_ERR_NO_DEVICE, "device %d out of range (%d present)",
              device, n);
    L2Z_HIP(hipSetDevice(device));
    if (g_cus == 0) {
        hipDeviceProp_t p;
        L2Z_HIP(hipGetDeviceProperties(&p, device));
        g_cus = p.multiProcessorCount > 0 ? p.multiProcessorCount : 256;
    }
    return L2Z_OK;
}

int current_device_for(const l2z_comm *comm)
{
    if (comm) return comm->device;
    int d = 0;
    if (hipGetDevice(&d) != hipSuccess) d = 0;
    return d;
}

}

using namespace l2z;

namespace {

constexpr size_t kBlobSlackFloats = 1024;
bool is_w1(const TensorDesc &d) { return strcmp(d.name, "w1") == 0; }
bool is_w3(const TensorDesc &d) { return strcmp(d.name, "w3") == 0; }

bool col_shard(const l2z_weights *w, const TensorDesc &d, size_t *c0, size_t *cl, size_t *cpad)
{
    if (!w->sh.scheme_b || d.kind != BY_DIM_ROWS) return false;
    const bool is_wo = strcmp(d.name, "wo") == 0;
    *c0 = is_wo ? w->sh.dim0 : w->sh.hid0;
    *cl = is_wo ? w->sh.dim_loc : w->sh.hid_loc;
    *cpad = is_wo ? w->sh.dimc_pad : w->sh.hidc_pad;
    return true;
}

size_t slot_floats(const l2z_weights *w, const TensorDesc &d)
{
    size_t r0, r1;
    shard_rows(d, w->sh, &r0, &r1);
    if (d.kind == SKIP && !w->file_layout) return 0;
    if (is_w3(d)) return 0;
    size_t c0, cl, cpad;
    if (col_shard(w, d, &c0, &cl, &cpad)) return d.layers * d.rows * cpad;
    return d.layers * (r1 - r0) * d.cols * (is_w1(d) ? 2 : 1);
}

void carve_local(l2z_weights *w, const std::vector<TensorDesc> &tt)
{
    size_t off = 0, off_w1 = 0;
    const float *base = w->blob;
    w->dev_off.assign(tt.size(), 0);
    for (size_t i = 0; i < tt.size(); i++) {
        const auto &d = tt[i];
        if (is_w1(d)) off_w1 = off;
        w->dev_off[i] = is_w3(d) ? off_w1 + d.cols : off;
        const float *p = base + w->dev_off[i];
        const std::string n = d.name;
        if (n == "token_embedding_table") w->tok_emb = p;
        else if (n == "rms_att_weight") w->rms_att = p;
        else if (n == "wq") w->wq = p;
        else if (n == "wk") w->wk = p;
        else if (n == "wv") w->wv = p;
        else if (n == "wo") w->wo = p;
        else if (n == "rms_ffn_weight") w->rms_ffn = p;
        else if (n == "w1") w->w1 = p;
        else if (n == "w2") w->w2 = p;
        else if (n == "w3") w->w3 = p;
        else if (n == "rms_final_weight") w->rms_final = p;
        else if (n == "wcls") w->wcls = p;
        off += slot_floats(w, d);
    }
    if (w->shared) w->wcls = w->tok_emb + (size_t)w->sh.v0 * w->cfg.dim;
}

size_t local_floats(const l2z_weights *w, const std::vector<TensorDesc> &tt)
{
    size_t off = 0;
    for (const auto &d : tt) off += slot_floats(w, d);
    return off;
}

hipError_t upload(float *dst, const float *src, size_t n_floats)
{
    const size_t piece = (size_t)256 << 20;
    hipError_t e = hipSuccess;
    for (size_t o = 0; o < n_floats && e == hipSuccess; o += piece) {
        const size_t n = n_floats - o < piece ? n_floats - o : piece;
        e = hipMemcpy(dst + o, src + o, n * sizeof(float), hipMemcpyHostToDevice);
    }
    return e;
}

int weights_alloc(const l2z_config *config, int shared_weights, const l2z_comm *comm,
                  l2z_weights **out, std::vector<TensorDesc> *tt_out)
{
    L2Z_CHECK(config != nullptr && out != nullptr, L2Z_ERR_INVALID, "weights_init: null argument");
    const int dev = current_device_for(comm);
    L2Z_TRY(ensure_device(dev));
    Shard sh;
    L2Z_TRY(make_shard(*config, comm, &sh));
    static std::atomic<uint64_t> next_uid{1};
    l2z_weights *w = new l2z_weights();
    w->uid = next_uid.fetch_add(1);
    w->cfg = *config;
    w->shared = shared_weights ? 1 : 0;
    w->device = dev;
    w->sh = sh;
    w->file_layout = sh.world == 1 && !sh.scheme_b;
    *tt_out = tensor_table(*config, w->shared != 0);
    w->blob_floats = local_floats(w, *tt_out);
    hipError_t e = hipMalloc(&w->blob, (w->blob_floats + kBlobSlackFloats) * sizeof(float));
    if (e == hipSuccess) e = hipMemset(w->blob + w->blob_floats, 0, kBlobSlackFloats * sizeof(float));
    if (e != hipSuccess) {
        set_error("hipMalloc(%zu bytes) for weights failed: %s", w->blob_floats * sizeof(float),
                  hipGetErrorString(e));
        delete w;
        return e == hipErrorOutOfMemory ? L2Z_ERR_OOM : L2Z_ERR_HIP;
    }
    carve_local(w, *tt_out);
    *out = w;
    return L2Z_OK;
}

void build_packed(l2z_weights *w)
{
    if (tunables().packed_w == 0 || !w->file_layout) return;
    const l2z_config &c = w->cfg;
    const size_t dim = c.dim, hid = c.hidden_dim;
    const int rows = 2 * c.hidden_dim, cols = c.dim, L = c.n_layers;
    if (!pk::width_ok(cols)) return;
    w->pk.assign(L, l2z_weights::PkMat{});
    w->pk_candidates = L;
    auto slot = [&](int l) { return w->w1 + (size_t)l * hid * 2 * dim; };
    std::vector<uint32_t> stats(3 * (size_t)L);
    for (int l = 0; l < L; l++) {
        stats[3 * l] = 0;
        stats[3 * l + 1] = 255;
        stats[3 * l + 2] = 0;
    }
    uint32_t *d_stats = nullptr;
    hipError_t e = hipMalloc((void **)&d_stats, stats.size() * sizeof(uint32_t));
    if (e == hipSuccess) e = hipMemcpy(d_stats, stats.data(), stats.size() * sizeof(uint32_t), hipMemcpyHostToDevice);
    for (int l = 0; l < L && e == hipSuccess; l++) e = launch_pk_stats(slot(l), (size_t)rows * cols, d_stats + 3 * l, nullptr);
    if (e == hipSuccess) e = hipMemcpy(stats.data(), d_stats, stats.size() * sizeof(uint32_t), hipMemcpyDeviceToHost);
    if (d_stats) (void)hipFree(d_stats);
    const size_t per = (size_t)(rows / 2) * pk::pair_dw(cols / 4);
    size_t total = 0;
    for (int l = 0; l < L; l++) total += pk::encodable(stats[3 * l], stats[3 * l + 1], stats[3 * l + 2]) ? per : 0;
    if (e == hipSuccess && total > 0) {
        e = hipMalloc((void **)&w->pk_blob, total * sizeof(uint32_t));
        if (e != hipSuccess) w->pk_blob = nullptr;
    }
    size_t off = 0;
    for (int l = 0; l < L && e == hipSuccess && w->pk_blob; l++) {
        if (!pk::encodable(stats[3 * l], stats[3 * l + 1], stats[3 * l + 2])) continue;
        e = launch_pk_pack(slot(l), rows, cols, (int)stats[3 * l], w->pk_blob + off, nullptr);
        w->pk[l].p = w->pk_blob + off;
        w->pk[l].e = (int)stats[3 * l];
        w->pk_packed++;
        off += per;
    }
    if (e == hipSuccess) e = hipDeviceSynchronize();
    if (e != hipSuccess) {
        (void)hipGetLastError();
        if (w->pk_blob) (void)hipFree(w->pk_blob);
        w->pk_blob = nullptr;
        w->pk.assign(L, l2z_weights::PkMat{});
        w->pk_packed = 0;
    }
}

}

extern "C" int l2z_abi_version(void) { return L2Z_ABI_VERSION; }
extern "C" const char *l2z_last_error(void) { return l2z::g_err; }

extern "C" int l2z_device_count(int *out_n)
{
    L2Z_CHECK(out_n != nullptr, L2Z_ERR_INVALID, "l2z_device_count: null out");
    int n = 0;
    hipError_t e = hipGetDeviceCount(&n);
    if (e != hipSuccess) n = 0;
    *out_n = n;
    return L2Z_OK;
}

extern "C" int l2z_device_info(int dev, char *name, size_t cap, int *out_cus, uint64_t *out_hbm)
{
    L2Z_TRY(ensure_device(dev));
    hipDeviceProp_t p;
    L2Z_HIP(hipGetDeviceProperties(&p, dev));
    if (name && cap) snprintf(name, cap, "%s (%s)", p.name[0] ? p.name : "AMD GPU", p.gcnArchName);
    if (out_cus) *out_cus = p.multiProcessorCount;
    if (out_hbm) *out_hbm = (uint64_t)p.totalGlobalMem;
    return L2Z_OK;
}

extern "C" int l2z_weights_init(const l2z_config *config, const float *data, size_t n_floats,
                                int shared_weights, const l2z_comm *comm, l2z_weights **out)
{
    L2Z_CHECK(data != nullptr, L2Z_ERR_INVALID, "l2z_weights_init: null data");
    std::vector<TensorDesc> tt;
    l2z_weights *w = nullptr;
    L2Z_TRY(weights_alloc(config, shared_weights, comm, &w, &tt));
    const size_t need = tt.back().offset + tt.back().count();
    if (n_floats < need) {
        set_error("l2z_weights_init: blob has %zu f32, config needs %zu", n_floats, need);
        l2z_weights_free(w);
        return L2Z_ERR_INVALID;
    }
    hipError_t e = hipSuccess;
    float *stage = nullptr;
    for (size_t i = 0; i < tt.size() && e == hipSuccess; i++) {
        const auto &d = tt[i];
        if (d.kind == SKIP && !w->file_layout) continue;
        size_t r0, r1;
        shard_rows(d, w->sh, &r0, &r1);
        const size_t rl = r1 - r0;
        float *dst = w->blob + w->dev_off[i];
        size_t c0, cl, cpad;
        if (col_shard(w, d, &c0, &cl, &cpad)) {
            e = hipMemset(dst, 0, d.layers * d.rows * cpad * sizeof(float));
            for (size_t l = 0; l < d.layers && e == hipSuccess; l++)
                e = hipMemcpy2D(dst + l * d.rows * cpad, cpad * sizeof(float), data + d.offset + l * d.rows * d.cols + c0,
                                d.cols * sizeof(float), cl * sizeof(float), d.rows, hipMemcpyHostToDevice);
            continue;
        }
        if (is_w1(d) || is_w3(d)) {
            const size_t piece_rows = std::max<size_t>(1, std::min<size_t>(rl, ((size_t)64 << 20) / (d.cols * sizeof(float))));
            if (stage == nullptr) e = hipMalloc((void **)&stage, 2 * piece_rows * d.cols * sizeof(float));
            size_t n_piece = 0;
            for (size_t l = 0; l < d.layers && e == hipSuccess; l++) {
                for (size_t r = 0; r < rl && e == hipSuccess; r += piece_rows, n_piece++) {
                    const size_t nr = std::min(piece_rows, rl - r);
                    float *sb = stage + (n_piece & 1) * piece_rows * d.cols;
                    e = upload(sb, data + d.offset + (l * d.rows + r0 + r) * d.cols, nr * d.cols);
                    if (e == hipSuccess) e = launch_copy_rows(dst + (l * rl + r) * 2 * d.cols, 2 * d.cols, sb, nr, d.cols, nullptr);
                }
            }
            if (e == hipSuccess) e = hipDeviceSynchronize();
        } else if (rl == d.rows) {
            e = upload(dst, data + d.offset, d.count());
        } else {
            for (size_t l = 0; l < d.layers && e == hipSuccess; l++)
                e = upload(dst + l * rl * d.cols, data + d.offset + (l * d.rows + r0) * d.cols, rl * d.cols);
        }
    }
    if (stage) (void)hipFree(stage);
    if (e != hipSuccess) {
        set_error("weight upload failed: %s", hipGetErrorString(e));
        l2z_weights_free(w);
        return L2Z_ERR_HIP;
    }
    build_packed(w);
    *out = w;
    return L2Z_OK;
}

extern "C" int l2z_weights_init_synthetic(const l2z_config *config, int shared_weights,
                                          uint64_t seed, const l2z_comm *comm, l2z_weights **out)
{
    std::vector<TensorDesc> tt;
    l2z_weights *w = nullptr;
    L2Z_TRY(weights_alloc(config, shared_weights, comm, &w, &tt));
    hipError_t e = hipSuccess;
    for (size_t i = 0; i < tt.size(); i++) {
        const auto &d = tt[i];
        if (d.kind == SKIP && !w->file_layout) continue;
        size_t r0, r1;
        shard_rows(d, w->sh, &r0, &r1);
        const size_t rl = r1 - r0;
        const bool pair = is_w1(d) || is_w3(d);
        size_t c0, cl, cpad;
        if (col_shard(w, d, &c0, &cl, &cpad)) {
            float *dst = w->blob + w->dev_off[i];
            e = hipMemsetAsync(dst, 0, d.layers * d.rows * cpad * sizeof(float), nullptr);
            for (size_t l = 0; l < d.layers && e == hipSuccess; l++)
                e = launch_synth_fill(dst + l * d.rows * cpad, d.offset + l * d.rows * d.cols + c0, d.rows * cl, seed, d.scale, d.bias,
                                      nullptr, cl, cpad, d.cols);
            continue;
        }
        for (size_t l = 0; l < d.layers && e == hipSuccess; l++) {
            const uint64_t base = d.offset + (l * d.rows + r0) * d.cols;
            e = launch_synth_fill(w->blob + w->dev_off[i] + l * rl * d.cols * (pair ? 2 : 1), base, rl * d.cols, seed, d.scale,
                                  d.bias, nullptr, pair ? d.cols : 0, pair ? 2 * d.cols : 0);
        }
    }
    if (e == hipSuccess) e = hipDeviceSynchronize();
    if (e != hipSuccess) {
        set_error("synthetic weight fill failed: %s", hipGetErrorString(e));
        l2z_weights_free(w);
        return L2Z_ERR_HIP;
    }
    build_packed(w);
    *out = w;
    return L2Z_OK;
}

extern "C" int l2z_weights_read(const l2z_weights *w, size_t offset, size_t count, float *out)
{
    L2Z_CHECK(w != nullptr && out != nullptr, L2Z_ERR_INVALID, "l2z_weights_read: null argument");
    L2Z_CHECK(w->file_layout, L2Z_ERR_INVALID, "l2z_weights_read: only for unsharded weights");
    L2Z_CHECK(offset + count <= w->blob_floats, L2Z_ERR_INVALID, "l2z_weights_read: out of range");
    L2Z_HIP(hipSetDevice(w->device));
    const std::vector<TensorDesc> tt = tensor_table(w->cfg, w->shared != 0);
    const size_t lo = offset, hi = offset + count;
    for (size_t i = 0; i < tt.size(); i++) {
        const auto &d = tt[i];
        const size_t t0 = std::max(lo, d.offset), t1 = std::min(hi, d.offset + d.count());
        if (t0 >= t1) continue;
        if (!(is_w1(d) || is_w3(d))) {
            L2Z_HIP(hipMemcpy(out + (t0 - lo), w->blob + w->dev_off[i] + (t0 - d.offset), (t1 - t0) * sizeof(float),
                              hipMemcpyDeviceToHost));
            continue;
        }
        for (size_t f = t0; f < t1;) {
            const size_t r = (f - d.offset) / d.cols, c = (f - d.offset) % d.cols;
            const float *src = w->blob + w->dev_off[i] + r * 2 * d.cols + c;
            const size_t whole = c == 0 ? (t1 - f) / d.cols : 0;
            if (whole > 0) {
                L2Z_HIP(hipMemcpy2D(out + (f - lo), d.cols * sizeof(float), src, 2 * d.cols * sizeof(float),
                                    d.cols * sizeof(float), whole, hipMemcpyDeviceToHost));
                f += whole * d.cols;
            } else {
                const size_t n = std::min(d.cols - c, t1 - f);
                L2Z_HIP(hipMemcpy(out + (f - lo), src, n * sizeof(float), hipMemcpyDeviceToHost));
                f += n;
            }
        }
    }
    return L2Z_OK;
}

extern "C" void l2z_weights_free(l2z_weights *w)
{
    if (!w) return;
    if (w->blob) (void)hipFree(w->blob);
    if (w->pk_blob) (void)hipFree(w->pk_blob);
    delete w;
}

extern "C" int l2z_weights_packed_count(const l2z_weights *w, int *n_packed, int *n_candidates)
{
    L2Z_CHECK(w != nullptr && n_packed != nullptr && n_candidates != nullptr, L2Z_ERR_INVALID,
              "l2z_weights_packed_count: null argument");
    *n_packed = w->pk_packed;
    *n_candidates = w->pk_candidates;
    return L2Z_OK;
}

extern "C" int l2z_weights_packed_read(const l2z_weights *w, int layer, float *out, size_t n_floats)
{
    L2Z_CHECK(w != nullptr && out != nullptr, L2Z_ERR_INVALID, "l2z_weights_packed_read: null argument");
    L2Z_CHECK(layer >= 0 && (size_t)layer < w->pk.size(), L2Z_ERR_INVALID, "l2z_weights_packed_read: no packed layer %d", layer);
    const auto &pm = w->pk[layer];
    L2Z_CHECK(pm.p != nullptr, L2Z_ERR_STATE, "l2z_weights_packed_read: layer %d is not packed", layer);
    const int rows = 2 * w->cfg.hidden_dim, cols = w->cfg.dim;
    const size_t count = (size_t)rows * cols;
    L2Z_CHECK(n_floats >= count, L2Z_ERR_INVALID, "l2z_weights_packed_read: need %zu floats", count);
    L2Z_HIP(hipSetDevice(w->device));
    float *d = nullptr;
    L2Z_HIP(hipMalloc((void **)&d, count * sizeof(float)));
    hipError_t e = launch_pk_unpack(pm.p, rows, cols, pm.e, d, nullptr);
    if (e == hipSuccess) e = hipMemcpy(out, d, count * sizeof(float), hipMemcpyDeviceToHost);
    (void)hipFree(d);
    L2Z_HIP(e);
    return L2Z_OK;
}
```

Measured before the change: 235.8 tokens/s.

## Extend packed weight encoding to QKV, WO, FFN2 and classifier matvecs

Packed (compressed, lossless-when-encodable) weight storage, previously used only for the fused w1/w3 FFN matvec, is now built per kind for QKV (three slots per layer), WO, FFN2 and the classifier. The row matvec kernel gains a two-register-set software pipeline that issues the next batch's packed load before decoding the current one, and ROPE picks per-segment packed pointers and exponents. The goal is to cut weight bytes read from HBM in every memory-bound matvec. In exchange it adds more decode ALU work, higher register pressure, extra packing time and memory at load, and disables push on packed launches.

```diff
diff --git a/llama2.zig_amd/csrc/forward.cpp b/llama2.zig_amd/csrc/forward.cpp
--- a/llama2.zig_amd/csrc/forward.cpp
+++ b/llama2.zig_amd/csrc/forward.cpp
@@ -137,7 +137,10 @@
         *epi = sh.rank == 0 ? EPI_RESID : EPI_STORE;
         push_to(a, 1);
     };
-    const bool pk = s->packed_w && w->pk_blob != nullptr && !sb && sh.world == 1 && !consume;
+    const bool pk = s->packed_w && !sb && sh.world == 1 && !consume;
+    const auto pk_slot = [&](int k, int l, int j = 0) -> const l2z_weights::PkMat * {
+        return pk && ((s->packed_kinds >> k) & 1) ? w->pk_slot(k, l, j) : nullptr;
+    };
     for (int l = 0; l < c.n_layers; l++) {
         float *kc = s->key_cache + (size_t)l * c.seq_len * sh.kvd_loc;
         float *vc = s->value_cache + (size_t)l * c.seq_len * sh.kvd_loc;
@@ -165,6 +168,12 @@
             a.n = c.dim; a.rms_w = w->rms_att + (size_t)l * dim;
             x_in(a, s->x, gi, sh.dim_loc);
             a.pos_ptr = s->d_pos; a.rope = s->rope; a.head_size = sh.hs; a.rope_segs = 2;
+            const auto *pq = pk_slot(KIND_QKV, l, 0), *pkk = pk_slot(KIND_QKV, l, 1), *pv = pk_slot(KIND_QKV, l, 2);
+            if (pq && pkk && pv) {
+                a.pk = pq->p; a.pk_e = pq->e;
+                a.pk1 = pkk->p; a.pk_e1 = pkk->e;
+                a.pk2 = pv->p; a.pk_e2 = pv->e;
+            }
             L2Z_LAUNCH(KIND_QKV, launch_matvec(a, PRO_RMS, EPI_ROPE, mb, g_cus, st));
         }
         if (!fused && want() && kind(KIND_ATTN)) {
@@ -197,6 +206,7 @@
                 a.rows0 = sh.dim_loc; a.n = c.dim;
                 x_in(a, s->xb, gi, sh.dim_loc);
                 push_to(a, 1);
+                if (const auto *p = pk_slot(KIND_WO, l)) { a.pk = p->p; a.pk_e = p->e; }
             }
             L2Z_LAUNCH(KIND_WO, launch_matvec(a, PRO_NONE, epi, mb, g_cus, st, nullptr, &pushed));
         }
@@ -211,7 +221,7 @@
             a.rms_w = w->rms_ffn + (size_t)l * dim;
             x_in(a, s->x, gi, sh.dim_loc);
             if (!sb) push_to(a, 2);
-            if (pk && w->pk[l].p != nullptr) { a.pk = w->pk[l].p; a.pk_e = w->pk[l].e; }
+            if (const auto *p = pk_slot(KIND_FFN13, l)) { a.pk = p->p; a.pk_e = p->e; }
             L2Z_LAUNCH(KIND_FFN13, launch_matvec(a, PRO_RMS, EPI_SWIGLU, mb, g_cus, st, nullptr, &pushed));
         }
         if (!sb) L2Z_TRY(gather(s->hb, sh.hid_loc));
@@ -226,6 +236,7 @@
                 a.rows0 = sh.dim_loc; a.n = c.hidden_dim;
                 x_in(a, s->hb, gi, sh.hid_loc);
                 push_to(a, 1);
+                if (const auto *p = pk_slot(KIND_FFN2, l)) { a.pk = p->p; a.pk_e = p->e; }
             }
             L2Z_LAUNCH(KIND_FFN2, launch_matvec(a, PRO_NONE, epi, mb, g_cus, st, nullptr, &pushed));
         }
@@ -242,6 +253,7 @@
                           matvec_vector_width(c.dim);
         int grid = 0;
         if (!xchg) push_to(a, 3);
+        if (const auto *p = fuse ? pk_slot(KIND_CLS, 0) : nullptr) { a.pk = p->p; a.pk_e = p->e; }
         L2Z_LAUNCH(KIND_CLS, launch_matvec(a, PRO_RMS, fuse ? EPI_ARGMAX : EPI_STORE, mb, g_cus, st,
                                            &grid, &pushed));
         s->n_part = fuse ? grid : 0;
diff --git a/llama2.zig_amd/csrc/l2z_internal.h b/llama2.zig_amd/csrc/l2z_internal.h
--- a/llama2.zig_amd/csrc/l2z_internal.h
+++ b/llama2.zig_amd/csrc/l2z_internal.h
@@ -115,8 +115,9 @@
     const int *push_ctl;
     int push_gi;
     LLIn xin;
-    const uint32_t *pk;
-    int pk_e;
+    const uint32_t *pk, *pk1, *pk2;
+    int pk_e, pk_e1, pk_e2;
+    int tl_slot;
 };
 
 struct AttnArgs {
diff --git a/llama2.zig_amd/csrc/l2z_state.h b/llama2.zig_amd/csrc/l2z_state.h
--- a/llama2.zig_amd/csrc/l2z_state.h
+++ b/llama2.zig_amd/csrc/l2z_state.h
@@ -44,6 +44,8 @@
 int current_device_for(const l2z_comm *comm);
 
 }
+
+enum { KIND_QKV = 0, KIND_ATTN, KIND_WO, KIND_FFN13, KIND_FFN2, KIND_CLS, KIND_ARGMAX, KIND_GATHER, KIND_COUNT };
 
 struct l2z_weights {
     uint64_t uid = 0;
@@ -61,10 +63,22 @@
     struct PkMat {
         const uint32_t *p = nullptr;
         int e = 0;
+        const float *src = nullptr;
+        int rows = 0, cols = 0;
     };
-    uint32_t *pk_blob = nullptr;
-    std::vector<PkMat> pk;
-    int pk_packed = 0, pk_candidates = 0;
+    struct PkKind {
+        uint32_t *blob = nullptr;
+        std::vector<PkMat> slots;
+        int per_layer = 0;
+        int packed = 0;
+    };
+    PkKind pk[KIND_COUNT];
+    const PkMat *pk_slot(int kind, int layer, int j = 0) const
+    {
+        const PkKind &k = pk[kind];
+        const size_t i = (size_t)layer * k.per_layer + j;
+        return k.blob != nullptr && i < k.slots.size() && k.slots[i].p != nullptr ? &k.slots[i] : nullptr;
+    }
 };
 
 struct l2z_kvpool {
@@ -76,7 +90,6 @@
     int live = 0;
 };
 
-enum { KIND_QKV = 0, KIND_ATTN, KIND_WO, KIND_FFN13, KIND_FFN2, KIND_CLS, KIND_ARGMAX, KIND_GATHER, KIND_COUNT };
 static const char *const kKindNames[KIND_COUNT] = {"qkv", "attn", "wo", "ffn13", "ffn2", "cls", "argmax", "gather"};
 static_assert(KIND_COUNT == L2Z_N_KINDS, "include/llama2_hip_test.h L2Z_N_KINDS");
 
@@ -138,6 +151,7 @@
     bool fused_qkv_attn = false;
     int max_blocks = 0;
     bool packed_w = true;
+    int packed_kinds = -1;
     int tl_attn_seq = 0;
     l2z::BatchScratch *bt = nullptr;
     float *rg_k = nullptr, *rg_v = nullptr;
diff --git a/llama2.zig_amd/csrc/matvec.hip b/llama2.zig_amd/csrc/matvec.hip
--- a/llama2.zig_amd/csrc/matvec.hip
+++ b/llama2.zig_amd/csrc/matvec.hip
@@ -199,13 +199,14 @@
 
 template <int EPI, int XC>
 struct RowF32 {
-    static constexpr bool kAhead = false;
+    static constexpr int kSets = 1;
     v4f wa[kRowU], wb[kRowU];
     const float *pa, *pb;
     int n4;
 
     __device__ __forceinline__ void init(const MvLocals &, int n4_, int) { n4 = n4_; }
     __device__ __forceinline__ void point(const MvLocals &m, int u) { pair_rows<EPI>(m, u, pa, pb); }
+    template <int P>
     __device__ __forceinline__ void issue(int b)
     {
         const int tid = threadIdx.x, cb = b * (kBlock * kRowU);
@@ -224,64 +225,83 @@
             wb[k] = ldg_nt(b4 + off);
         }
     }
+    template <int P>
     __device__ __forceinline__ void deliver() {}
 };
 
-template <int XC>
+template <int EPI, int XC>
 struct RowPacked {
-    static constexpr bool kAhead = true;
+    static constexpr int kSets = 2;
     v4f wa[kRowU], wb[kRowU];
-    PkRaw raw, nraw;
-    int s_cur, s_nxt;
+    PkRaw raw[kSets];
+    int s_in[kSets], e31[kSets];
     const uint32_t *pp;
     size_t pdw, last_off;
-    int e31, s_last, wave_u, n_batches;
-
-    __device__ __forceinline__ void init(const MvLocals &m, int n4, int n_batches_)
+    int e_pt, s_last, wave_u, n_batches;
+
+    __device__ __forceinline__ void init(const MvLocals &, int n4, int n_batches_)
     {
         n_batches = n_batches_;
-        e31 = m.pk_e - 31;
         wave_u = __builtin_amdgcn_readfirstlane(threadIdx.x >> 6);
         pdw = pk::pair_dw(n4);
         last_off = pk::chunk_off(n4, n_batches - 1, wave_u);
         s_last = pk::steps(n4, n_batches - 1, wave_u);
     }
-    __device__ __forceinline__ void point(const MvLocals &m, int u) { pp = pair_packed(m, u, pdw); }
+    __device__ __forceinline__ void point(const MvLocals &m, int u)
+    {
+        int e;
+        pp = pair_packed<EPI>(m, u, pdw, e);
+        e_pt = e - 31;
+    }
+    template <int P>
     __device__ __forceinline__ void issue(int b)
     {
         const bool last = b + 1 == n_batches;
         const uint32_t *src = pp + (last ? last_off : (size_t)b * (4 * 64 * pk::kMaxLaneDw) + (size_t)wave_u * (64 * pk::kMaxLaneDw));
-        s_nxt = (XC == 4 || !last) ? 4 : s_last;
-        pk_load_raw(src, threadIdx.x & 63, XC == 4 ? 4 : s_nxt, nraw);
-    }
-    __device__ __forceinline__ void rotate()
-    {
-        raw = nraw;
-        s_cur = s_nxt;
-    }
+        s_in[P] = (XC == 4 || !last) ? 4 : s_last;
+        e31[P] = e_pt;
+        pk_load_raw(src, threadIdx.x & 63, XC == 4 ? 4 : s_in[P], raw[P]);
+    }
+    template <int P>
     __device__ __forceinline__ void deliver()
     {
         if constexpr (XC == 4) {
-            pk_decode_lane<4>(raw, e31, wa, wb);
+            pk_decode_lane<4>(raw[P], e31[P], wa, wb);
         } else {
-            switch (s_cur) {
-                case 4: pk_decode_lane<4>(raw, e31, wa, wb); break;
-                case 3: pk_decode_lane<3>(raw, e31, wa, wb); break;
-                case 2: pk_decode_lane<2>(raw, e31, wa, wb); break;
-                case 1: pk_decode_lane<1>(raw, e31, wa, wb); break;
-                default: pk_decode_lane<0>(raw, e31, wa, wb); break;
+            switch (s_in[P]) {
+                case 4: pk_decode_lane<4>(raw[P], e31[P], wa, wb); break;
+                case 3: pk_decode_lane<3>(raw[P], e31[P], wa, wb); break;
+                case 2: pk_decode_lane<2>(raw[P], e31[P], wa, wb); break;
+                case 1: pk_decode_lane<1>(raw[P], e31[P], wa, wb); break;
+                default: pk_decode_lane<0>(raw[P], e31[P], wa, wb); break;
             }
         }
     }
 };
+
+#ifdef L2Z_TIMELINE
+constexpr int kMtlSlots = 256, kMtlBlocks = 512;
+__device__ long long g_mtl[kMtlSlots * kMtlBlocks * 8];
+unsigned long long g_mtl_launches = 0;
+#define L2Z_MTL(i) tl[i] = wall_clock64()
+#else
+#define L2Z_MTL(i) do { } while (0)
+#endif
 
 template <int PRO, int EPI, int XC, bool LL, bool PK = false>
 __global__ __launch_bounds__(kBlock) void matvec_row_kernel(const MatvecArgs a)
 {
     constexpr int U = kRowU;
-    using Src = typename std::conditional<PK, RowPacked<XC>, RowF32<EPI, XC>>::type;
+    using Src = typename std::conditional<PK, RowPacked<EPI, XC>, RowF32<EPI, XC>>::type;
+    constexpr int NS = Src::kSets;
     extern __shared__ __attribute__((aligned(16))) float lds[];
-    const MvLocals m = mv_locals<EPI>(a);
+#ifdef L2Z_TIMELINE
+    long long tl[8] = {0, 0, 0, 0, 0, 0, 0, 0};
+#endif
+    L2Z_MTL(0);
+    MvLocals m_ = mv_locals<EPI>(a);
+    if constexpr (PK) m_.push = nullptr;
+    const MvLocals m = m_;
     const int n4 = m.n >> 2;
     const int n_batches = (n4 + kBlock * U - 1) / (kBlock * U);
     const int n4_pad = n_batches * (kBlock * U);
@@ -301,33 +321,58 @@
     src.point(m, u);
     EpiIn ein = epi_prefetch<EPI>(m, u, tid == 0);
     EpiIn ein_next = ein;
-    src.issue(0);
-    if constexpr (Src::kAhead) src.rotate();
+    src.template issue<0>(0);
+    L2Z_MTL(1);
     xst.finish(a.x, a.rms_w, m.n, n4_pad, xs, scratch);
+    L2Z_MTL(2);
+
+    int iu = u, ib = 0;
+    bool imore = true;
+    auto advance = [&]() __attribute__((always_inline)) {
+        const MvStep s = mv_step(iu, ib, n_batches, ustride, n_units);
+        imore = s.more;
+        if (s.more) {
+            if (s.unit_done) src.point(m, s.u_next);
+            iu = s.u_next;
+            ib = s.b_next;
+        }
+    };
+    advance();
 
     v4f acc_a = {0.f, 0.f, 0.f, 0.f}, acc_b = {0.f, 0.f, 0.f, 0.f};
     ArgmaxCand best;
     int b = 0, parity = 0;
-    while (true) {
+    auto step = [&](auto set, auto ahead) __attribute__((always_inline)) -> bool {
+        constexpr int P = decltype(set)::value;
         const MvStep s = mv_step(u, b, n_batches, ustride, n_units);
-        auto issue_next = [&]() __attribute__((always_inline)) {
-            if (s.more) {
-                if (s.unit_done) {
-                    src.point(m, s.u_next);
-                    ein_next = epi_prefetch<EPI>(m, s.u_next, tid == 0);
-                }
-                src.issue(s.b_next);
-            }
+        auto prefetch_next = [&]() __attribute__((always_inline)) {
+            if (s.more && s.unit_done) ein_next = epi_prefetch<EPI>(m, s.u_next, tid == 0);
         };
-        if constexpr (Src::kAhead) issue_next();
-        src.deliver();
+        if constexpr (NS > 1) {
+            prefetch_next();
+            if constexpr (decltype(ahead)::value) {
+                if constexpr (EPI == EPI_SWIGLU) asm volatile("s_waitcnt vmcnt(0)" ::: "memory");
+                src.template issue<(P + 1) % NS>(ib);
+                advance();
+            }
+        }
+        src.template deliver<P>();
 #pragma unroll
         for (int k = 0; k < U; k++) {
             const v4f xv = xs4[b * (kBlock * U) + tid + kBlock * k];
             acc_a = fma4(src.wa[k], xv, acc_a);
             acc_b = fma4(src.wb[k], xv, acc_b);
         }
-        if constexpr (!Src::kAhead) issue_next();
+        if constexpr (NS == 1) {
+            prefetch_next();
+            if (imore) {
+                src.template issue<0>(ib);
+                advance();
+            }
+        }
+#ifdef L2Z_TIMELINE
+        tl[6]++;
+#endif
         if (s.unit_done) {
             const float sa = wave_sum(hsum4(acc_a));
             const float sb = wave_sum(hsum4(acc_b));
@@ -351,16 +396,39 @@
             parity ^= 1;
             acc_a = v4f{0.f, 0.f, 0.f, 0.f};
             acc_b = v4f{0.f, 0.f, 0.f, 0.f};
-        }
-        if (!s.more) break;
-        if constexpr (Src::kAhead) src.rotate();
+#ifdef L2Z_TIMELINE
+            if (tl[7]++ == 0) L2Z_MTL(3);
+            L2Z_MTL(4);
+#endif
+        }
         u = s.u_next;
         b = s.b_next;
+        return !s.more;
+    };
+    using Set0 = std::integral_constant<int, 0>;
+    using Set1 = std::integral_constant<int, 1>;
+    static_assert(NS == 1 || NS == 2, "register sets of a source");
+    if constexpr (NS == 1) {
+        while (!step(Set0{}, std::false_type{})) {}
+    } else {
+        while (true) {
+            if (!imore) { step(Set0{}, std::false_type{}); break; }
+            step(Set0{}, std::true_type{});
+            if (!imore) { step(Set1{}, std::false_type{}); break; }
+            step(Set1{}, std::true_type{});
+        }
     }
     if (EPI == EPI_ARGMAX && tid == 0) {
         a.part_val[blockIdx.x] = best.v;
         a.part_idx[blockIdx.x] = best.i;
     }
+#ifdef L2Z_TIMELINE
+    L2Z_MTL(5);
+    if (tid == 0 && (unsigned)a.tl_slot < (unsigned)kMtlSlots && blockIdx.x < kMtlBlocks) {
+        long long *o = g_mtl + ((size_t)a.tl_slot * kMtlBlocks + blockIdx.x) * 8;
+        for (int i = 0; i < 8; i++) o[i] = tl[i];
+    }
+#endif
 }
 
 template <int PRO, int EPI>
@@ -417,11 +485,11 @@
 
 #define L2Z_MV_COMBOS(X)                     \
     X(PRO_NONE, EPI_STORE,  0, 1, 0)         \
-    X(PRO_NONE, EPI_RESID,  1, 1, 0)         \
+    X(PRO_NONE, EPI_RESID,  1, 1, 1)         \
     X(PRO_RMS,  EPI_STORE,  1, 1, 0)         \
-    X(PRO_RMS,  EPI_ROPE,   1, 1, 0)         \
+    X(PRO_RMS,  EPI_ROPE,   1, 1, 1)         \
     X(PRO_RMS,  EPI_SWIGLU, 1, 1, 1)         \
-    X(PRO_RMS,  EPI_ARGMAX, 1, 0, 0)
+    X(PRO_RMS,  EPI_ARGMAX, 1, 0, 1)
 #define L2Z_IF_1(...) __VA_ARGS__
 #define L2Z_IF_0(...)
 
@@ -510,6 +578,10 @@
     const bool ll = a.xin.slots != nullptr;
     if (ll && !vec) return hipErrorNotSupported;
     if (a.pk != nullptr && (!use_row || ll || !pk::width_ok(a.n))) return hipErrorInvalidValue;
+    if (a.pk != nullptr) a.push = nullptr;
+    if (a.pk != nullptr && epi != EPI_SWIGLU &&
+        ((a.rows1 > 0 && a.pk1 == nullptr) || (a.rows2 > 0 && a.pk2 == nullptr) || a.rows0 % 2 || a.rows1 % 2 || a.rows2 % 2))
+        return hipErrorInvalidValue;
     MvLaunch k = {nullptr, 0, 0};
     size_t lds;
     int n_units;
@@ -559,8 +631,21 @@
     if (out_grid) *out_grid = grid;
     if (!vec || epi == EPI_ROPE || a.rows2 != 0 || (epi != EPI_SWIGLU && a.rows1 != 0)) a.push = nullptr;
     if (pushed) *pushed = a.push != nullptr;
+#ifdef L2Z_TIMELINE
+    a.tl_slot = use_row ? (int)(g_mtl_launches++ % kMtlSlots) : -1;
+#endif
     void *args[] = {&a};
     return hipLaunchKernel(k.fn, dim3(grid), dim3(kBlock), args, lds, st);
 }
 
 }
+
+#ifdef L2Z_TIMELINE
+extern "C" int l2z_matvec_timeline_dump(long long *out, unsigned long long *n_launches)
+{
+    if (hipDeviceSynchronize() != hipSuccess) return 1;
+    if (hipMemcpyFromSymbol(out, HIP_SYMBOL(l2z::g_mtl), sizeof(long long) * l2z::kMtlSlots * l2z::kMtlBlocks * 8) != hipSuccess) return 1;
+    *n_launches = l2z::g_mtl_launches;
+    return 0;
+}
+#endif
diff --git a/llama2.zig_amd/csrc/matvec_device.h b/llama2.zig_amd/csrc/matvec_device.h
--- a/llama2.zig_amd/csrc/matvec_device.h
+++ b/llama2.zig_amd/csrc/matvec_device.h
@@ -15,8 +15,8 @@
     const P2pArgs *push;
     int push_e;
     size_t push_base;
-    const uint32_t *pk;
-    int pk_e;
+    const uint32_t *pk, *pk1, *pk2;
+    int pk_e, pk_e1, pk_e2;
 };
 
 template <int EPI>
@@ -36,7 +36,8 @@
     m.push = a.push;
     m.push_e = m.push ? a.push_ctl[kCtlEpoch] + a.push_gi : 0;
     m.push_base = m.push ? (size_t)m.push->rank * m.push->count : 0;
-    m.pk = a.pk; m.pk_e = a.pk_e;
+    m.pk = a.pk; m.pk1 = a.pk1; m.pk2 = a.pk2;
+    m.pk_e = a.pk_e; m.pk_e1 = a.pk_e1; m.pk_e2 = a.pk_e2;
     return m;
 }
 
@@ -77,9 +78,16 @@
     }
 }
 
-__device__ __forceinline__ const uint32_t *pair_packed(const MvLocals &m, int p, size_t pair_dw)
+template <int EPI>
+__device__ __forceinline__ const uint32_t *pair_packed(const MvLocals &m, int p, size_t pair_dw, int &e_base)
 {
     if (p >= m.n_pairs) p = m.n_pairs - 1;
+    if (EPI == EPI_ROPE) {
+        const SegRow r = seg_row(m, 2 * p);
+        e_base = r.pick(m.pk_e, m.pk_e1, m.pk_e2);
+        return r.pick(m.pk, m.pk1, m.pk2) + (size_t)(r.row >> 1) * pair_dw;
+    }
+    e_base = m.pk_e;
     return m.pk + (size_t)p * pair_dw;
 }
 
diff --git a/llama2.zig_amd/csrc/runstate.cpp b/llama2.zig_amd/csrc/runstate.cpp
--- a/llama2.zig_amd/csrc/runstate.cpp
+++ b/llama2.zig_amd/csrc/runstate.cpp
@@ -34,6 +34,7 @@
     s->max_blocks = tn.max_blocks_per_cu;
     s->use_graphs = tn.no_graph == 0;
     s->packed_w = tn.packed_w != 0;
+    s->packed_kinds = tn.packed_kinds;
     if (comm && comm->world > 1 && !comm->nccl && !comm->p2p) s->use_graphs = false;
     s->fused_qkv_attn = sh.world == 1 && tn.fuse_small != 0 &&
                         fused_qkv_attn_supported(c.dim, c.n_heads, c.n_kv_heads, c.seq_len, g_cus);
diff --git a/llama2.zig_amd/csrc/tunables.cpp b/llama2.zig_amd/csrc/tunables.cpp
--- a/llama2.zig_amd/csrc/tunables.cpp
+++ b/llama2.zig_amd/csrc/tunables.cpp
@@ -35,6 +35,7 @@
     env_int("L2Z_PF_X3_STREAM_MIN", &t.pf_x3_stream_min);
     env_int("L2Z_PF_FUSE_PLANES", &t.pf_fuse_planes);
     env_int("L2Z_PACKED_W", &t.packed_w);
+    env_int("L2Z_PACKED_KINDS", &t.packed_kinds);
     return t;
 }
 
@@ -74,7 +75,8 @@
         {"L2Z_P2P_BULK_MB", &t.p2p_bulk_mb}, {"L2Z_PREFILL", &t.prefill}, {"L2Z_PF_CHUNK", &t.pf_chunk},
         {"L2Z_PF_PANEL", &t.pf_panel}, {"L2Z_PF_PANEL_MAX", &t.pf_panel_max},
         {"L2Z_PF_X3", &t.pf_x3}, {"L2Z_PF_X3_STREAM_MIN", &t.pf_x3_stream_min},
-        {"L2Z_PF_FUSE_PLANES", &t.pf_fuse_planes}, {"L2Z_PACKED_W", &t.packed_w}};
+        {"L2Z_PF_FUSE_PLANES", &t.pf_fuse_planes}, {"L2Z_PACKED_W", &t.packed_w},
+        {"L2Z_PACKED_KINDS", &t.packed_kinds}};
     for (auto &e : ints)
         if (strcmp(e.n, name) == 0) {
             *e.p = (int)v;
diff --git a/llama2.zig_amd/csrc/tunables.h b/llama2.zig_amd/csrc/tunables.h
--- a/llama2.zig_amd/csrc/tunables.h
+++ b/llama2.zig_amd/csrc/tunables.h
@@ -21,6 +21,7 @@
     int pf_x3_stream_min = 33;
     int pf_fuse_planes = 1;
     int packed_w = 1;
+    int packed_kinds = -1;
     int pf_panel_max = -1;
 
     static constexpr int row_blocks = 2;
diff --git a/llama2.zig_amd/csrc/weights.cpp b/llama2.zig_amd/csrc/weights.cpp
--- a/llama2.zig_amd/csrc/weights.cpp
+++ b/llama2.zig_amd/csrc/weights.cpp
@@ -240,51 +240,87 @@
     return L2Z_OK;
 }
 
-void build_packed(l2z_weights *w)
-{
-    if (tunables().packed_w == 0 || !w->file_layout) return;
-    const l2z_config &c = w->cfg;
-    const size_t dim = c.dim, hid = c.hidden_dim;
-    const int rows = 2 * c.hidden_dim, cols = c.dim, L = c.n_layers;
-    if (!pk::width_ok(cols)) return;
-    w->pk.assign(L, l2z_weights::PkMat{});
-    w->pk_candidates = L;
-    auto slot = [&](int l) { return w->w1 + (size_t)l * hid * 2 * dim; };
-    std::vector<uint32_t> stats(3 * (size_t)L);
-    for (int l = 0; l < L; l++) {
-        stats[3 * l] = 0;
-        stats[3 * l + 1] = 255;
-        stats[3 * l + 2] = 0;
+void build_packed_kind(l2z_weights *w, int kind, int per_layer, std::vector<l2z_weights::PkMat> slots)
+{
+    l2z_weights::PkKind &k = w->pk[kind];
+    k.per_layer = per_layer;
+    k.slots = std::move(slots);
+    const size_t n = k.slots.size();
+    std::vector<uint32_t> stats(3 * n);
+    for (size_t i = 0; i < n; i++) {
+        stats[3 * i] = 0;
+        stats[3 * i + 1] = 255;
+        stats[3 * i + 2] = 0;
     }
     uint32_t *d_stats = nullptr;
     hipError_t e = hipMalloc((void **)&d_stats, stats.size() * sizeof(uint32_t));
     if (e == hipSuccess) e = hipMemcpy(d_stats, stats.data(), stats.size() * sizeof(uint32_t), hipMemcpyHostToDevice);
-    for (int l = 0; l < L && e == hipSuccess; l++) e = launch_pk_stats(slot(l), (size_t)rows * cols, d_stats + 3 * l, nullptr);
+    for (size_t i = 0; i < n && e == hipSuccess; i++)
+        e = launch_pk_stats(k.slots[i].src, (size_t)k.slots[i].rows * k.slots[i].cols, d_stats + 3 * i, nullptr);
     if (e == hipSuccess) e = hipMemcpy(stats.data(), d_stats, stats.size() * sizeof(uint32_t), hipMemcpyDeviceToHost);
     if (d_stats) (void)hipFree(d_stats);
-    const size_t per = (size_t)(rows / 2) * pk::pair_dw(cols / 4);
+    const auto dwords = [&](size_t i) -> size_t {
+        const auto &m = k.slots[i];
+        if (m.rows % 2 || !pk::encodable(stats[3 * i], stats[3 * i + 1], stats[3 * i + 2])) return 0;
+        return (size_t)(m.rows / 2) * pk::pair_dw(m.cols / 4);
+    };
     size_t total = 0;
-    for (int l = 0; l < L; l++) total += pk::encodable(stats[3 * l], stats[3 * l + 1], stats[3 * l + 2]) ? per : 0;
+    for (size_t i = 0; i < n; i++) total += dwords(i);
     if (e == hipSuccess && total > 0) {
-        e = hipMalloc((void **)&w->pk_blob, total * sizeof(uint32_t));
-        if (e != hipSuccess) w->pk_blob = nullptr;
+        e = hipMalloc((void **)&k.blob, total * sizeof(uint32_t));
+        if (e != hipSuccess) k.blob = nullptr;
     }
     size_t off = 0;
-    for (int l = 0; l < L && e == hipSuccess && w->pk_blob; l++) {
-        if (!pk::encodable(stats[3 * l], stats[3 * l + 1], stats[3 * l + 2])) continue;
-        e = launch_pk_pack(slot(l), rows, cols, (int)stats[3 * l], w->pk_blob + off, nullptr);
-        w->pk[l].p = w->pk_blob + off;
-        w->pk[l].e = (int)stats[3 * l];
-        w->pk_packed++;
-        off += per;
+    for (size_t i = 0; i < n && e == hipSuccess && k.blob; i++) {
+        auto &m = k.slots[i];
+        if (dwords(i) == 0) continue;
+        e = launch_pk_pack(m.src, m.rows, m.cols, (int)stats[3 * i], k.blob + off, nullptr);
+        m.p = k.blob + off;
+        m.e = (int)stats[3 * i];
+        k.packed++;
+        off += dwords(i);
     }
     if (e == hipSuccess) e = hipDeviceSynchronize();
     if (e != hipSuccess) {
         (void)hipGetLastError();
-        if (w->pk_blob) (void)hipFree(w->pk_blob);
-        w->pk_blob = nullptr;
-        w->pk.assign(L, l2z_weights::PkMat{});
-        w->pk_packed = 0;
+        if (k.blob) (void)hipFree(k.blob);
+        k.blob = nullptr;
+        for (auto &m : k.slots) m.p = nullptr;
+        k.packed = 0;
+    }
+}
+
+void build_packed(l2z_weights *w)
+{
+    if (tunables().packed_w == 0 || !w->file_layout) return;
+    const l2z_config &c = w->cfg;
+    const size_t dim = c.dim, hid = c.hidden_dim, kvd = (size_t)c.dim / c.n_heads * c.n_kv_heads;
+    const int L = c.n_layers;
+    using Slots = std::vector<l2z_weights::PkMat>;
+    const auto mat = [](const float *src, size_t rows, size_t cols) {
+        l2z_weights::PkMat m;
+        m.src = src; m.rows = (int)rows; m.cols = (int)cols;
+        return m;
+    };
+    if (pk::width_ok(c.dim)) {
+        Slots s13, sqkv, so, scls;
+        for (int l = 0; l < L; l++) {
+            s13.push_back(mat(w->w1 + (size_t)l * hid * 2 * dim, 2 * hid, dim));
+            sqkv.push_back(mat(w->wq + (size_t)l * dim * dim, dim, dim));
+            sqkv.push_back(mat(w->wk + (size_t)l * kvd * dim, kvd, dim));
+            sqkv.push_back(mat(w->wv + (size_t)l * kvd * dim, kvd, dim));
+            so.push_back(mat(w->wo + (size_t)l * dim * dim, dim, dim));
+        }
+        scls.push_back(mat(w->wcls, c.vocab_size, dim));
+        build_packed_kind(w, KIND_FFN13, 1, std::move(s13));
+        build_packed_kind(w, KIND_QKV, 3, std::move(sqkv));
+        build_packed_kind(w, KIND_WO, 1, std::move(so));
+        build_packed_kind(w, KIND_CLS, 1, std::move(scls));
+    }
+    if (pk::width_ok(c.hidden_dim)) {
+        Slots s2;
+        for (int l = 0; l < L; l++) s2.push_back(mat(w->w2 + (size_t)l * dim * hid, dim, hid));
+        build_packed_kind(w, KIND_FFN2, 1, std::move(s2));
     }
 }
 
@@ -454,34 +490,59 @@
 {
     if (!w) return;
     if (w->blob) (void)hipFree(w->blob);
-    if (w->pk_blob) (void)hipFree(w->pk_blob);
+    for (auto &k : w->pk)
+        if (k.blob) (void)hipFree(k.blob);
     delete w;
 }
 
-extern "C" int l2z_weights_packed_count(const l2z_weights *w, int *n_packed, int *n_candidates)
-{
-    L2Z_CHECK(w != nullptr && n_packed != nullptr && n_candidates != nullptr, L2Z_ERR_INVALID,
-              "l2z_weights_packed_count: null argument");
-    *n_packed = w->pk_packed;
-    *n_candidates = w->pk_candidates;
-    return L2Z_OK;
-}
-
-extern "C" int l2z_weights_packed_read(const l2z_weights *w, int layer, float *out, size_t n_floats)
-{
-    L2Z_CHECK(w != nullptr && out != nullptr, L2Z_ERR_INVALID, "l2z_weights_packed_read: null argument");
-    L2Z_CHECK(layer >= 0 && (size_t)layer < w->pk.size(), L2Z_ERR_INVALID, "l2z_weights_packed_read: no packed layer %d", layer);
-    const auto &pm = w->pk[layer];
-    L2Z_CHECK(pm.p != nullptr, L2Z_ERR_STATE, "l2z_weights_packed_read: layer %d is not packed", layer);
-    const int rows = 2 * w->cfg.hidden_dim, cols = w->cfg.dim;
-    const size_t count = (size_t)rows * cols;
+namespace {
+
+int packed_read_slot(const l2z_weights *w, int kind, int layer, int j, float *out, size_t n_floats)
+{
+    const l2z_weights::PkKind &k = w->pk[kind];
+    L2Z_CHECK(layer >= 0 && j >= 0 && j < k.per_layer && (size_t)layer * k.per_layer + j < k.slots.size(), L2Z_ERR_INVALID,
+              "l2z_weights_packed_read: no packed slot %d of layer %d of kind %s", j, layer, kKindNames[kind]);
+    const l2z_weights::PkMat *pm = w->pk_slot(kind, layer, j);
+    L2Z_CHECK(pm != nullptr, L2Z_ERR_STATE, "l2z_weights_packed_read: slot %d of layer %d of kind %s is not packed", j, layer,
+              kKindNames[kind]);
+    const size_t count = (size_t)pm->rows * pm->cols;
     L2Z_CHECK(n_floats >= count, L2Z_ERR_INVALID, "l2z_weights_packed_read: need %zu floats", count);
     L2Z_HIP(hipSetDevice(w->device));
     float *d = nullptr;
     L2Z_HIP(hipMalloc((void **)&d, count * sizeof(float)));
-    hipError_t e = launch_pk_unpack(pm.p, rows, cols, pm.e, d, nullptr);
+    hipError_t e = launch_pk_unpack(pm->p, pm->rows, pm->cols, pm->e, d, nullptr);
     if (e == hipSuccess) e = hipMemcpy(out, d, count * sizeof(float), hipMemcpyDeviceToHost);
     (void)hipFree(d);
     L2Z_HIP(e);
     return L2Z_OK;
 }
+
+}
+
+extern "C" int l2z_weights_packed_count(const l2z_weights *w, int *n_packed, int *n_candidates)
+{
+    return l2z_weights_packed_count_kind(w, KIND_FFN13, n_packed, n_candidates);
+}
+
+extern "C" int l2z_weights_packed_read(const l2z_weights *w, int layer, float *out, size_t n_floats)
+{
+    L2Z_CHECK(w != nullptr && out != nullptr, L2Z_ERR_INVALID, "l2z_weights_packed_read: null argument");
+    return packed_read_slot(w, KIND_FFN13, layer, 0, out, n_floats);
+}
+
+extern "C" int l2z_weights_packed_count_kind(const l2z_weights *w, int kind, int *n_packed, int *n_candidates)
+{
+    L2Z_CHECK(w != nullptr && n_packed != nullptr && n_candidates != nullptr, L2Z_ERR_INVALID,
+              "l2z_weights_packed_count: null argument");
+    L2Z_CHECK(kind >= 0 && kind < KIND_COUNT, L2Z_ERR_INVALID, "l2z_weights_packed_count_kind: bad kind %d", kind);
+    *n_packed = w->pk[kind].packed;
+    *n_candidates = (int)w->pk[kind].slots.size();
+    return L2Z_OK;
+}
+
+extern "C" int l2z_weights_packed_read_kind(const l2z_weights *w, int kind, int layer, int slot, float *out, size_t n_floats)
+{
+    L2Z_CHECK(w != nullptr && out != nullptr, L2Z_ERR_INVALID, "l2z_weights_packed_read: null argument");
+    L2Z_CHECK(kind >= 0 && kind < KIND_COUNT, L2Z_ERR_INVALID, "l2z_weights_packed_read_kind: bad kind %d", kind);
+    return packed_read_slot(w, kind, layer, slot, out, n_floats);
+}
```

Measured after the change: 242.9 tokens/s, median of 6. 3.0% higher.
